# crowsonkb/style-transfer-pytorch

Hardware: AMD Instinct MI355X
Metric: optimizer iterations/sec (higher is better)
Workload: dtype f32 (3x3 convs: fp16x3 split-plane MFMA, fp32 accumulate); 1 GPU; 512x512 single-scale hot loop (closure + Adam + clamp + EMA), 1 style image 512x512, VGG-19 synthetic weights, max pooling; parallelism=single GPU

## Files before the change

include/st_amd.h:

```cpp
#ifndef ST_AMD_H
#define ST_AMD_H

#ifdef __cplusplus
extern "C" {
#endif

#define ST_AMD_ABI_VERSION 2

#define ST_NUM_CONVS 13
#define ST_NUM_STYLE_LAYERS 5
#define ST_CONTENT_LAYER 22
#define ST_NUM_LOSS_TERMS 7

enum st_pooling { ST_POOL_MAX = 0, ST_POOL_AVERAGE = 1, ST_POOL_L2 = 2 };

typedef struct st_net st_net;
typedef struct st_plan st_plan;

const char* st_last_error(void);
int st_abi_version(void);
const char* st_compiled_arch(void);
int st_has_experiments(void);
int st_env_switches(const char** names, int capacity);
int st_set_option(const char* name, int value, int clear);
// ... 70 lines not shown

typedef struct st_exchange {
    int kind;
    long long count;
    float* send_up;
    float* send_down;
    float* recv_up;
    float* recv_down;
    float* buffer;
    int root;
    int channel;
    void* stream;
} st_exchange;
int st_plan_create_strip(st_plan** out, const st_net* net, int global_height, int width, int row_begin,
                         int row_end);
int st_plan_set_rank(st_plan* plan, int rank, int world);
int st_plan_closure_begin(st_plan* plan, const float* image, float* grad_out);
int st_plan_closure_next(st_plan* plan, st_exchange* exchange, void* stream);

typedef struct st_fabric st_fabric;
int st_fabric_unique_id(unsigned char* id128);
int st_fabric_create(st_fabric** out, const unsigned char* id_trunk128, const unsigned char* id_heads128, int rank, int world,
                     int self_halo);
int st_fabric_destroy(st_fabric* fabric);
int st_fabric_abort(st_fabric* fabric);
int st_fabric_selftest(st_fabric* fabric, void* stream, int timeout_ms);
int st_plan_closure_run(st_plan* plan, st_fabric* fabric, void* stream);
long long st_qn_strip_state_bytes(long long count, int world);
int st_qn_strip_dots(void* state, long long count, int rank, int world, const float* grad, st_exchange* gather,
                     void* stream);
int st_qn_strip_apply(void* state, long long count, int world, float* image, const float* grad, float* ema_value,
                      double ema_decay, void* stream);
int st_plan_qn_strip_step(st_plan* plan, st_fabric* fabric, float* image, float* grad, void* state, float* ema_value,
                          double ema_decay, void* stream);
int st_plan_losses(st_plan* plan, float** losses);
int st_plan_term_losses(st_plan* plan, float** terms, int* count);
int st_plan_forward_begin(st_plan* plan, const float* image, int last_layer);
int st_plan_moment_sums(st_plan* plan, int layer, float* sums, void* stream);

int st_plan_set_graph(st_plan* plan, int enable);

int st_plan_profile_enable(st_plan* plan, int enable);
int st_plan_profile_read(st_plan* plan, long long* launches, double* millis, double* flops);
int st_plan_profile_read_hbm(st_plan* plan, int category, long long* launches, double* millis, double* bytes);

int st_op_sqrtm_ns(const float* a, float* root, int n, void* stream);
int st_op_sqrtm_ns_backward(const float* root, const float* grad_root, float* grad_a, int n, void* stream);
int st_op_sqrtm_ns_backward_diag(const float* root, float grad_diag, float* grad_a, int n, void* stream);
int st_op_tv_loss(const float* image, int height, int width, float* loss_out, float* grad_out, void* stream);
int st_op_conv3x3(const float* in, const float* weight, const float* bias, float* out, int cin, int cout,
                  int height, int width, int relu, int precision, void* stream);
int st_op_conv3x3_dgrad(const float* grad_out, const float* relu_out, const float* weight, float* grad_in,
                        int cin, int cout, int height, int width, int precision, void* stream);
int st_op_conv3x3_strip(const float* in, const float* halo, int has_up, int has_down, const float* weight,
                        const float* bias, float* out, int cin, int cout, int height, int width, int relu, int dgrad,
                        int precision, void* stream);
int st_op_conv3x3_strip_ex(const float* in, const float* halo, int has_up, int has_down, const float* weight,
                           const float* bias, float* out, const float* out_mask, int cin, int cout, int height, int width,
                           int relu, int dgrad, int accumulate, int overlap, int precision, void* stream);

int st_op_conv1x1(const float* in, const float* weight, const float* bias, float* out, int cin, int cout,
                  long long npix, int precision, void* stream);

int st_op_pool2x2(const float* in, float* out, int channels, int height, int width, int mode, void* stream);
int st_op_pool2x2_backward(const float* in, const float* grad_out, float* grad_in, int channels, int height, int width,
                           int mode, void* stream);


typedef struct st_head st_head;
int st_head_create(st_head** out, int kind, int channels, int height, int width, int precision);
int st_head_destroy(st_head* head);
long long st_head_device_bytes(const st_head* head);
long long st_head_state_floats(const st_head* head);
int st_head_moments(st_head* head, const float* feat, float* mean_out, float* srm_out, void* stream);
int st_head_forward(st_head* head, const float* feat, const float* mean_t, const float* cov_t, const float* root_t,
                    const float* gram_t, float eps, float* loss_out, float* state, void* stream);
int st_head_backward(st_head* head, const float* feat, const float* state, const float* upstream, float* grad_feat,
                     void* stream);

long long st_op_reduce_scratch_floats(void);
int st_op_mse_loss(const float* x, const float* target, long long count, float* scratch, float* loss_out, void* stream);
int st_op_mse_loss_backward(const float* x, const float* target, long long count, const float* upstream, float* grad,
                            void* stream);
int st_op_scaled_mse_loss(const float* x, const float* target, long long count, float eps, float* scratch, float* totals,
                          float* loss_out, void* stream);
int st_op_scaled_mse_loss_backward(const float* x, const float* target, long long count, const float* totals,
                                   const float* upstream, float* grad, void* stream);
int st_op_tv_value(const float* image, int height, int width, float* scratch, float* loss_out, void* stream);
int st_op_tv_loss_backward(const float* image, int height, int width, const float* upstream, float* grad, void* stream);


int st_op_sqrtm_time(int n, int iters, double* fwd_us, double* bwd_us, void* stream);

int st_op_conv3x3_time(int cin, int cout, int height, int width, int dgrad, int precision, int iters,
                       double* avg_us, void* stream);

int st_op_mfma_rate(int lds_reads, int waves, int steps, int launches, double* tflops, double* mhz, void* stream);

int st_op_mfma_valu_rate(int lds_reads, int waves, int steps, int launches, int valu_waves, int valu_steps,
                         int valu_prio, double* tflops, double* mhz, double* cycles, void* stream);

int st_op_winograd_consumer_rate(int steps, int launches, double* tflops, void* stream);

int st_plan_debug_read(st_plan* plan, int what, float* out, int count);

int st_op_grid_barrier_time(int workgroups, int rounds, int payload_floats, int groups, double* us_per_round, int* errors,
                            void* stream);

#ifdef __cplusplus
}
#endif
#endif
```

style-transfer-pytorch_amd/csrc/st_api.hip:

```cpp
#include <atomic>
#include <cmath>
#include <cstdlib>
#include <cstring>
#include <mutex>
#include <vector>

#include "st_plan.h"

namespace st {

static thread_local std::string g_error;
void set_error(const char* fmt, ...) {
    char buf[1024];
    va_list ap;
    va_start(ap, fmt);
    vsnprintf(buf, sizeof(buf), fmt, ap);
    va_end(ap);
    g_error = buf;
}
const char* get_error() { return g_error.c_str(); }

static std::mutex g_option_mutex;
static std::vector<std::pair<std::string, int>> g_option_override;
static std::atomic<unsigned> g_option_gen{1};
// ... 467 lines not shown
        if (p->net->conv_elem == 1) { tail.zero = reinterpret_cast<unsigned int*>(p->amax_word); tail.zero_count = 64ll * kAmaxWordUints; }
    }
    const AdamScalars sc = adam_scalars(step, lr, beta1, beta2, eps, ema_decay);
    FoldUpdate upd{image, exp_avg, exp_avg_sq, ema_value, sc, tail};
    if (upd.tail.losses_copy == upd.tail.losses8) upd.tail.losses_copy = nullptr;
    p->defer_sum = fold_tail;
    p->fold_update = fold_step ? &upd : nullptr;
    p->fold_updated = false;
    const int closure_rc = closure_entry(p, image, p->grad_img, losses_out, s);
    p->defer_sum = false;
    p->fold_update = nullptr;
    if (closure_rc) return 1;
    if (p->fold_updated) {
        p->fold_updated = false;
        p->amax_clean = tail.zero != nullptr;
        return 0;
    }
    const int rc = hbm_profiled(p, HBM_ADAM, 9.0 * 3 * 4.0 * p->H * p->W, s, [&] {
        return launch_adam_clamp_ema(image, p->grad_img, exp_avg, exp_avg_sq, ema_value, 3ll * p->H * p->W, sc, s, tail);
    });
    p->amax_clean = rc == 0 && tail.zero != nullptr;
    return rc;
}

int st_plan_apply_update(st_plan* p, float* image, const float* grad, float* exp_avg, float* exp_avg_sq,
                         float* ema_value, long long step, double lr, double beta1, double beta2, double eps,
                         double ema_decay, void* stream) {
    ST_REQUIRE(p && image && grad && exp_avg && exp_avg_sq && ema_value, "st_plan_apply_update: null argument");
    ST_REQUIRE(step >= 1, "st_plan_apply_update: step must be >= 1");
    return launch_adam_clamp_ema(image, grad, exp_avg, exp_avg_sq, ema_value, 3ll * p->H * p->W,
                                 adam_scalars(step, lr, beta1, beta2, eps, ema_decay),
                                 static_cast<hipStream_t>(stream));
}

int st_plan_debug_read(st_plan* p, int what, float* out, int count) {
    ST_REQUIRE(p && out && count > 0, "st_plan_debug_read: bad argument");
    const bool grad_map = what >= 16 && what < 16 + kNumOps;
    ST_REQUIRE((what == 0 && count <= 4 * kStreamBlocks) || (what == 1 && count <= kStreamBlocks * 256 * 5 && tv_debug_buffer()) ||
                   (what == 2 && count == 64) ||
                   (grad_map && p->grads_allocated && (size_t)count == node_at(p, what - 16).count()),
               "st_plan_debug_read: unknown buffer or count out of range");
    ST_HIP(hipDeviceSynchronize());
    if (what == 2) {
        std::vector<unsigned int> words((size_t)64 * kAmaxWordUints);
        ST_HIP(hipMemcpy(words.data(), p->amax_word, words.size() * sizeof(unsigned int), hipMemcpyDeviceToHost));
        for (int w = 0; w < 64; ++w) {
            unsigned int m = 0;
            for (int slot = 0; slot < kAmaxSlots; ++slot) m = std::max(m, words[(size_t)w * kAmaxWordUints + (size_t)slot * kAmaxSlotStride]);
            memcpy(&out[w], &m, sizeof(float));
        }
        return 0;
    }
    if (grad_map) {
        ST_HIP(hipMemcpy(out, node_at(p, what - 16).g, (size_t)count * sizeof(float), hipMemcpyDeviceToHost));
        return 0;
    }
    ST_HIP(hipMemcpy(out, what == 0 ? p->red_partials : tv_debug_buffer(), (size_t)count * sizeof(float), hipMemcpyDeviceToHost));
    return 0;
}

int st_plan_losses(st_plan* p, float** losses) {
    ST_REQUIRE(p && losses, "st_plan_losses: null argument");
    *losses = p->losses;
    return 0;
}

int st_plan_moment_sums(st_plan* p, int layer, float* sums, void* stream) {
    ST_REQUIRE(p && sums, "st_plan_moment_sums: null argument");
    int idx = -1;
    for (int k = 0; k < p->n_style; ++k)
        if (kProgram[p->style_op[k]].feat_index == layer) idx = k;
    ST_REQUIRE(idx >= 0, "st_plan_moment_sums: features[%d] is not a style layer", layer);
    if (ensure_style_alloc(p, p->head[p->style_op[idx]], p->style_kind[idx])) return 1;
    return moment_sums_of_tap(p, idx, sums, static_cast<hipStream_t>(stream));
}

int st_plan_set_graph(st_plan* p, int enable) {
    ST_REQUIRE(p, "st_plan_set_graph: null plan");
    p->graph_enabled = enable != 0;
    if (!enable) invalidate_graph(p);
    return 0;
}

int st_plan_profile_enable(st_plan* p, int enable) {
    ST_REQUIRE(p, "st_plan_profile_enable: null plan");
    p->profiling = enable != 0;
    return 0;
}

int st_plan_profile_read(st_plan* p, long long* launches, double* millis, double* flops) {
    ST_REQUIRE(p, "st_plan_profile_read: null plan");
    for (size_t i = 0; i < p->events_used; ++i) {
        ProfileEvent& e = p->events[i];
        ST_HIP(hipEventSynchronize(e.stop));
        float ms = 0.f;
        ST_HIP(hipEventElapsedTime(&ms, e.start, e.stop));
        p->prof_ms += ms;
        p->prof_flops += e.flops;
        p->prof_launches += 1;
    }
    p->events_used = 0;
    p->hbm_used = 0;
    if (launches) *launches = p->prof_launches;
    if (millis) *millis = p->prof_ms;
    if (flops) *flops = p->prof_flops;
    p->prof_launches = 0;
    p->prof_ms = 0;
    p->prof_flops = 0;
    return 0;
}
// ... 24 lines not shown
```

style-transfer-pytorch_amd/csrc/st_closure.hip:

```cpp
#include <cmath>
#include <cstdlib>
#include <mutex>

#include "st_plan.h"

namespace st {

void conv_arithmetic(const st_net* net, int conv, bool dgrad, ConvProblem& c) {
    const bool wide = dgrad ? net->wide_bwd[conv] : net->wide_fwd[conv];
    if (wide) {
        c.wgt_split = dgrad ? net->wsx_bwd[conv] : net->wsx_fwd[conv];
        c.planes = 3;
        c.elem = 0;
    } else {
        c.wgt_split = dgrad ? net->ws_bwd[conv] : net->ws_fwd[conv];
        c.planes = net->conv_planes;
        c.elem = net->conv_elem;
    }
}

int plan_alloc(st_plan* p, float** out, size_t floats) {
    void* ptr = nullptr;
    const size_t bytes = ((floats * sizeof(float) + 255) / 256) * 256;
    hipError_t e = hipMalloc(&ptr, bytes);
// ... 448 lines not shown
    return 0;
}

static bool head5_masks_its_gradient() {
    static Option opt("ST_HEAD5_MASK", 1);
    return opt.get() != 0;
}

int style_head_gradient(st_plan* p, const HeadSite& at, hipStream_t s) {
    StyleHead& h = *at.h;
    const Node& tap = *at.tap;
    const bool f16 = p->net->conv_elem == 1;
    static Option head_f32("ST_HEAD_1X1_F32", 0);
    const float* out_mask = (at.slot == 4 && head5_masks_its_gradient()) ? tap.y : nullptr;
    if (ablate_side() & 2) return 0;
    return hbm_profiled(p, HBM_HEAD_1X1, 2.0 * h.n * (double)tap.h * tap.w * sizeof(float), s, [&] {
        return head_step(h, tap.y, tap.h, tap.w, at.grad, s, f16 && !head_f32.get(), tap.y_amax, f16 ? at.grad_amax : nullptr, out_mask);
    });
}

bool op_is_tap(const st_plan* p, int op) {
    for (int i = 0; i < p->n_content; ++i)
        if (p->content_op[i] == op) return true;
    for (int k = 0; k < p->n_style; ++k)
        if (p->style_op[k] == op) return true;
    return false;
}

int join_head_for_conv(st_plan* p, int conv_index, hipStream_t s) {
    for (int k = 0; k < p->n_style; ++k) {
        if (!head_taps_conv(p, k, conv_index)) continue;
        ST_HIP(hipStreamWaitEvent(s, p->head_done[k], 0));
    }
    return 0;
}

void dgrad_conv(const st_plan* p, int i, ConvProblem& c) {
    const st_net* net = p->net;
    const OpDesc& op = kProgram[i];
    const OpDesc& pop = kProgram[i - 1];
    const Node& n = p->conv[op.index];
    const Node& in = node_at(p, i - 1);
    const bool top = i == kNumOps - 1;
    c.in = n.g; c.mask = (top && !head5_masks_its_gradient()) ? n.y : nullptr;
    c.out_mask = (pop.kind == 0) ? in.y : nullptr;
    c.wgt = net->w_bwd[op.index]; c.bias = nullptr; c.out = in.g;
    c.cin = op.cout; c.cout = op.cin; c.height = n.h; c.width = n.w; c.taps = 9; c.relu = 0;
    c.accumulate = (pop.kind == 0 && op_is_tap(p, i - 1)) ? 1 : 0;
    c.scratch = p->conv_scratch;
    conv_arithmetic(net, op.index, true, c);
    c.amax_word = n.g_amax; c.out_amax = net->conv_elem == 1 ? in.g_amax : nullptr;
}

int run_backward(st_plan* p, float* grad_image, hipStream_t s) {
    const st_net* net = p->net;
    for (int i = kNumOps - 1; i >= 0; --i) {
        const OpDesc& op = kProgram[i];
        if (op.kind == 0) {
            Node& n = p->conv[op.index];
            if (join_head_for_conv(p, op.index, s)) return 1;
            if (op.index == 0) {
                ST_HIP(hipStreamWaitEvent(s, p->tv_done, 0));
                if (hbm_profiled(p, HBM_CONV1_DGRAD, (64 + 3 + 3) * 4.0 * p->H * p->W, s, [&] {
                        return launch_conv_first_dgrad(n.g, nullptr, net->w_first, grad_image, p->dp_scratch, p->H, p->W, 1, s, nullptr, 0, 0,
                                                       p->dp_parts, p->fold_update);
                    }))
                    return 1;
                p->fold_updated = p->fold_update != nullptr;
                continue;
            }
            const OpDesc& pop = kProgram[i - 1];
            if (pop.kind == 0 && join_head_for_conv(p, pop.index, s)) return 1;
            if (i - 1 == p->content_op[0]) ST_HIP(hipStreamWaitEvent(s, p->content_done, 0));
            ConvProblem c{};
            dgrad_conv(p, i, c);
            if (conv_launch_profiled(p, c, s)) return 1;
        } else {
            Node& n = p->pool[op.index];
            const OpDesc& pop = kProgram[i - 1];
            Node& in = p->conv[pop.index];
            const double bytes = in.coded ? (in.count() + 1.25 * n.count()) * 4.0 : (2.0 * in.count() + n.count()) * 4.0;
            if (hbm_profiled(p, HBM_POOL_BWD, bytes, s, [&] {
                    if (in.coded) return launch_pool_bwd_codes(in.pool_code, n.g, in.g, in.c, in.h, in.w, s);
                    return launch_pool_bwd(in.y, n.g, in.g, in.c, in.h, in.w, net->pooling, s);
                }))
                return 1;
        }
    }
    return 0;
}

int run_tap_backward(st_plan* p, const float* const* seed, float* grad_image, hipStream_t s, bool onto_image) {
    const st_net* net = p->net;
    const bool bounds = net->conv_elem == 1;
    int top = -1;
    for (int i = 0; i < kNumOps; ++i)
        if (seed[i]) top = i;
    ST_REQUIRE(top >= 0, "st_plan_backward: no tap gradient given");
    if (bounds)
        ST_HIP(hipMemsetAsync(reinterpret_cast<unsigned int*>(p->amax_word) + (size_t)16 * kAmaxWordUints, 0,
                              (size_t)32 * kAmaxWordUints * sizeof(unsigned int), s));
    {
        Node& n = node_at(p, top);
        if (launch_seed_grad(seed[top], kProgram[top].kind == 0 ? n.y : nullptr, n.g, (long long)n.count(), 0,
                             bounds ? n.g_amax : nullptr, s))
            return 1;
    }
    for (int i = top; i >= 0; --i) {
        const OpDesc& op = kProgram[i];
        if (op.kind == 0 && op.index == 0) {
            if (hbm_profiled(p, HBM_CONV1_DGRAD, (64 + 3 + (onto_image ? 3 : 0)) * 4.0 * p->H * p->W, s, [&] {
                    return launch_conv_first_dgrad(p->conv[0].g, nullptr, net->w_first, grad_image, p->dp_scratch, p->H, p->W,
                                                   onto_image ? 1 : 0, s, nullptr, 0, 0, p->dp_parts,
                                                   onto_image ? p->fold_update : nullptr);
                }))
                return 1;
            if (onto_image) p->fold_updated = p->fold_update != nullptr;
            return 0;
        }
        Node& in = node_at(p, i - 1);
        const float* in_seed = seed[i - 1];
        if (op.kind == 0) {
            if (in_seed && launch_seed_grad(in_seed, nullptr, in.g, (long long)in.count(), 0, nullptr, s)) return 1;
            ConvProblem c{};
            dgrad_conv(p, i, c);
            c.mask = nullptr;
            c.accumulate = in_seed ? 1 : 0;
            if (conv_launch_profiled(p, c, s)) return 1;
        } else {
            Node& n = p->pool[op.index];
            if (hbm_profiled(p, HBM_POOL_BWD, (2.0 * in.count() + n.count()) * 4.0, s, [&] {
                    return launch_pool_bwd(in.y, n.g, in.g, in.c, in.h, in.w, net->pooling, s);
                }))
                return 1;
            if (in_seed && launch_seed_grad(in_seed, in.y, in.g, (long long)in.count(), 1, bounds ? in.g_amax : nullptr, s))
                return 1;
        }
    }
    return 0;
}

static bool shallow_heads_lockstep(const st_plan* p) {
    static Option opt("ST_HEAD_LOCKSTEP", 1);
    return opt.get() != 0 && p->net->conv_elem == 1;
}

int require_targets(const st_plan* p) {
    for (int i = 0; i < p->n_content; ++i)
        ST_REQUIRE(p->content_set[p->content_op[i]], "content target %d (features[%d]) not set (st_plan_set_content_target_at)", i,
                   kProgram[p->content_op[i]].feat_index);
    for (int j = 0; j < p->n_style; ++j)
        ST_REQUIRE(p->head[p->style_op[j]].target_set, "style target %d (features[%d]) not set (st_plan_set_style_target)", j,
                   kProgram[p->style_op[j]].feat_index);
    for (int r = 1; r < p->n_regions; ++r)
        for (int j = 0; j < p->n_style; ++j)
            ST_REQUIRE(p->region_head[r - 1][p->style_op[j]].target_set,
                       "style target %d (features[%d]) of region %d not set (st_plan_set_region_style_target)", j,
                       kProgram[p->style_op[j]].feat_index, r);
    return 0;
}

int loss_and_grad(st_plan* p, const float* image, float* grad_out, float* losses_out, hipStream_t s) {
    if (require_targets(p) || ensure_grad_alloc(p)) return 1;
    if (ensure_streams(p, s)) return 1;
    if (p->timeline) ST_HIP(hipEventRecord(p->tl_start, s));
    auto tv = [&](hipStream_t ts) {
        return hbm_profiled(p, HBM_TV, 2.0 * 3 * 4.0 * p->H * p->W, ts, [&] {
            return launch_tv(image, p->H, p->W, p->tv_weight, grad_out, p->red_partials, p->losses + 6, ts, p->tickets + 0);
        });
    };
    static Option tv_slot_opt("ST_TV_SLOT", 0);
    const bool tv_tail = tv_slot_opt.get() == 1 && !p->aux_stream;
    if (!tv_tail) {
        const int tvk = shallow_heads_lockstep(p) ? 2 : 0;
        if (!p->aux_stream && ensure_head_stream(p, tvk)) return 1;
        hipStream_t tvs = p->aux_stream ? p->aux_stream : p->head_stream[tvk];
        ST_HIP(hipEventRecord(p->aux_in, s));
        ST_HIP(hipStreamWaitEvent(tvs, p->aux_in, 0));
        if (tv(tvs)) return 1;
        ST_HIP(hipEventRecord(p->tv_done, tvs));
    }
    if (run_forward(p, image, 29, s, true)) return 1;
    if (p->timeline) ST_HIP(hipEventRecord(p->tl_fwd, s));
// ... 106 lines not shown
```

style-transfer-pytorch_amd/csrc/st_common.h:

```cpp
#pragma once

#include <hip/hip_runtime.h>

#include <algorithm>
#include <atomic>
#include <cstdarg>
#include <cstdio>
#include <string>

namespace st {

typedef float f32x16 __attribute__((ext_vector_type(16)));
typedef float f32x4 __attribute__((ext_vector_type(4)));
typedef float f32x2 __attribute__((ext_vector_type(2)));

constexpr int kWave = 64;

void set_error(const char* fmt, ...);
const char* get_error();

#define ST_HIP(expr)                                                                           \
    do {                                                                                       \
        hipError_t _e = (expr);                                                                \
        if (_e != hipSuccess) {                                                                \
// ... 71 lines not shown
};
__device__ __forceinline__ float w2_gdiag(const W2LossJob& j) { return -2.f * (j.weight / (float)j.n); }
__device__ __forceinline__ void w2_loss_block(const W2LossJob& j, float* scratch) {
#pragma clang fp contract(off)
    float sm = 0.f, sc = 0.f;
    for (int i = threadIdx.x; i < j.n; i += 256) {
        const float d = j.mean[i] - j.mean_t[i];
        sm += d * d;
        const size_t ii = (size_t)i * j.n + i;
        sc += (j.cov_t[ii] + j.cov[ii]) - 2.f * j.root[ii];
    }
    sm = block_sum_256(sm, scratch);
    sc = block_sum_256(sc, scratch);
    if (threadIdx.x == 0) {
        const float fn = (float)j.n;
        j.loss_out[0] = (sm / fn + sc / fn) * j.weight;
        j.gdiag_out[0] = w2_gdiag(j);
    }
}

static inline int ceil_div(int a, int b) { return (a + b - 1) / b; }

struct ConvProblem {
    const float* in;
    const float* mask;
    const float* wgt;
    const float* bias;
    float* out;
    int cin, cout, height, width;
    int taps;
    int relu;
    int accumulate;
    float* scratch;
    const float* in_halo;
    int has_up, has_down;
    int tune;
    const void* wgt_split;
    int planes;
    int elem;
    unsigned int* amax_word;
    int amax_measure;
    int halo_amax_folded;
    const unsigned int* halo_bound_up;
    const unsigned int* halo_bound_down;
    const unsigned int* wgt_amax;
    const float* out_mask;
    unsigned int* out_amax;
    int row_begin, row_end;
    int row_skip_begin, row_skip_len;
    int xcd_co_groups;
    int overlap_part;
    float* pool_out;
    unsigned char* pool_code;
    const void* wgt_wino;
    int wino;
};
constexpr int kAmaxSlots = 32;
constexpr int kAmaxSlotStride = 64;
constexpr int kAmaxWordUints = kAmaxSlots * kAmaxSlotStride;
#if defined(__HIPCC__)
__device__ __forceinline__ void amax_commit(unsigned int m, unsigned int* bound) {
#pragma unroll
    for (int off = 32; off >= 1; off >>= 1) {
        const unsigned int o = (unsigned int)__shfl_xor((int)m, off);
        m = o > m ? o : m;
    }
    unsigned int* slot = bound + (blockIdx.x % kAmaxSlots) * kAmaxSlotStride;
    if ((threadIdx.x & 63) == 0 && (m >> 23) > (*slot >> 23)) atomicMax(slot, m);
}
__device__ __forceinline__ unsigned int amax_read(const unsigned int* bound) {
    unsigned int m = bound[(threadIdx.x % kAmaxSlots) * kAmaxSlotStride];
#pragma unroll
    for (int off = 16; off >= 1; off >>= 1) {
        const unsigned int o = (unsigned int)__shfl_xor((int)m, off);
        m = o > m ? o : m;
    }
    return (unsigned int)__builtin_amdgcn_readfirstlane((int)m);
}
__device__ __forceinline__ unsigned int logical_block(int remap) {
    const unsigned int linear = blockIdx.y * gridDim.x + blockIdx.x, total = gridDim.x * gridDim.y;
    if (!remap || (total & 7u) != 0) return linear;
    return (linear & 7u) * (total >> 3) + (linear >> 3);
}
__device__ __forceinline__ unsigned int abs_bits(float v) { return __builtin_bit_cast(unsigned int, v) & 0x7fffffffu; }
__device__ __forceinline__ unsigned int amax_with_halo(unsigned int own, const unsigned int* up, const unsigned int* down) {
    if (up) { const unsigned int u = up[0] & 0x7fffffffu; own = u > own ? u : own; }
    if (down) { const unsigned int d = down[0] & 0x7fffffffu; own = d > own ? d : own; }
    return own;
}
__host__ __device__ __forceinline__ int scale_exp(unsigned int amax_bits) {
    const int ef = (int)((amax_bits >> 23) & 0xffu);
    if (ef == 0 || ef == 255) return 0;
    const int e = 14 - (ef - 126);
    return e > 120 ? 120 : (e < -120 ? -120 : e);
}
__device__ __forceinline__ float pow2f(int e) { return __builtin_bit_cast(float, (unsigned int)(127 + e) << 23); }
#endif
int launch_conv_split(const ConvProblem& p, hipStream_t stream);
#if defined(ST_EXPERIMENTS)
size_t winograd_weight_bytes(int cin, int cout);
int launch_winograd_weights(const float* w_torch, void* out, int cin, int cout, int dgrad, hipStream_t s);
bool conv_wino_applies(const ConvProblem& p);
bool conv_wino_preferred(const ConvProblem& p);
int launch_conv_wino(const ConvProblem& p, hipStream_t s);
#else
inline size_t winograd_weight_bytes(int, int) { return 256; }
inline int launch_winograd_weights(const float*, void*, int, int, int, hipStream_t) {
    set_error("the Winograd convolution (precision code 5) needs a library built with build.py --experiments");
    return 1;
}
inline bool conv_wino_applies(const ConvProblem&) { return false; }
inline bool conv_wino_preferred(const ConvProblem&) { return false; }
inline int launch_conv_wino(const ConvProblem&, hipStream_t) { return launch_winograd_weights(nullptr, nullptr, 0, 0, 0, nullptr); }
#endif
int launch_amax(const float* x, long long n, unsigned int* word, int single, hipStream_t s);
bool conv_pc_applies(const ConvProblem& p);
bool conv_pc_preferred(const ConvProblem& p);
int launch_conv_pc(const ConvProblem& p, hipStream_t stream);
bool conv_fat_applies(const ConvProblem& p);
bool conv_fat_preferred(const ConvProblem& p);
int launch_conv_fat(const ConvProblem& p, hipStream_t stream);
bool conv1x1_split_applies(const ConvProblem& p);
int launch_conv1x1_split(const ConvProblem& p, hipStream_t stream);
int launch_conv_splitk_reduce(const ConvProblem& p, int ksplit, hipStream_t stream);
inline bool conv_precision_valid(int code) { return code == 0 || code == 2 || code == 3 || code == 4; }
inline int conv_precision_planes(int code) { return code == 4 ? 2 : code; }
inline int conv_precision_elem(int code) { return code == 4 ? 1 : 0; }
inline size_t split_weight_bytes(int cin, int cout, int planes) { return (size_t)cin * cout * 9 * 2 * planes + 256; }
int launch_relayout_split(const float* w, void* out, int cin, int cout, int dgrad, int planes, int elem, hipStream_t s);
constexpr size_t kConvScratchFloats = (size_t)8 << 20;
int launch_conv(const ConvProblem& p, hipStream_t stream);
double conv_flops(const ConvProblem& p);

int launch_relayout_fwd(const float* w, float* out, int cin, int cout, hipStream_t stream);
int launch_relayout_dgrad(const float* w, float* out, int cin, int cout, hipStream_t stream);

constexpr int kPackScratchUints = 2 * 512 * 8 + 64;
int launch_pack_rows(const float* src, const float* mask, int channels, int height, int width, float* out_up,
                     float* out_down, hipStream_t s, unsigned int* bounds_up = nullptr, unsigned int* bounds_down = nullptr,
                     unsigned int* scratch = nullptr);

int launch_conv_first_fwd(const float* image, const float* w , const float* b, float* out,
                          int height, int width, hipStream_t stream, const float* halo = nullptr,
                          int has_up = 0, int has_down = 0, unsigned int* out_amax = nullptr);
bool conv_first_gram_applies(int height, int width, const float* image, const float* out, int max_splits);
int launch_conv_first_fwd_gram(const float* image, const float* w, const float* b, float* out, int height, int width,
                               hipStream_t stream, unsigned int* out_amax, float* partial, float* partial_sum, int max_splits,
                               int* splits, float w_l1max, float b_max);
int conv_first_dgrad_parts(int height, int width);
struct FoldUpdate;
int launch_conv_first_dgrad(const float* grad_out, const float* relu_out, const float* w, float* grad_image,
                            float* dp_scratch, int height, int width, int accumulate, hipStream_t stream,
                            const float* ghalo = nullptr, int has_up = 0, int has_down = 0, int parts = 1,
                            const FoldUpdate* update = nullptr);

int launch_pool_fwd(const float* in, float* out, int channels, int height, int width, int mode, hipStream_t s);
bool conv_pc_fuses_pool(const ConvProblem& p);
int fold_halo_amax(const ConvProblem& p, hipStream_t stream);
struct PcOverlap {
    int rows_b;
    int rows_bottom;
    int shape_i, tw_i;
    int shape_b, tw_b;
    double cost_split, cost_whole;
    bool pays;
    bool pool;
};
bool conv_pc_overlap_choice(const ConvProblem& p, PcOverlap* out);
int launch_pool_bwd_codes(const unsigned char* code, const float* grad_out, float* grad_in, int channels, int height,
                          int width, hipStream_t s);
// ... 273 lines not shown
```

style-transfer-pytorch_amd/csrc/st_conv.hip:

```cpp
#include <cstdlib>
#include <type_traits>

#include "st_common.h"

namespace st {

namespace {

constexpr int kChunk3x3 = 8, kChunk1x1 = 32;

template <int TAPS, int TW, int WN, int WGM>
struct Cfg {
    static constexpr int KC = (TAPS == 9) ? kChunk3x3 : kChunk1x1;
    static constexpr int WGN = 4 / WGM;
    static constexpr int TCO = 64 * WGM;
    static constexpr int NPIX = 32 * WN * WGN;
    static constexpr int TH = NPIX / TW;
    static constexpr int HALO = (TAPS == 9) ? 1 : 0;
    static constexpr int LH = TH + 2 * HALO;
    static constexpr int LW = TW + 2 * HALO;
    static constexpr int PLANE = LH * LW;
    static constexpr int NE_IN = KC * PLANE;
    static constexpr int IN_FLOATS = (NE_IN + 3) & ~3;
    static constexpr int NI = (NE_IN + 255) / 256;
// ... 358 lines not shown

long long padded_area(int h, int w, int th, int tw) {
    return (long long)ceil_div(h, th) * th * (long long)ceil_div(w, tw) * tw;
}

template <int WN, int WGM>
int launch_3x3(const ConvProblem& p, int ksplit, hipStream_t s) {
    constexpr int NPIX = 32 * WN * (4 / WGM);
    int best = 32;
    long long best_area = padded_area(p.height, p.width, NPIX / 32, 32);
    for (int tw : {16, 8}) {
        const long long a = padded_area(p.height, p.width, NPIX / tw, tw);
        if (a < best_area) { best_area = a; best = tw; }
    }
    if (best == 32) return launch_cfg<9, 32, WN, WGM>(p, ksplit, s);
    if (best == 16) return launch_cfg<9, 16, WN, WGM>(p, ksplit, s);
    return launch_cfg<9, 8, WN, WGM>(p, ksplit, s);
}

}

int launch_conv_splitk_reduce(const ConvProblem& p, int ksplit, hipStream_t stream) {
    const long long total = (long long)p.cout * p.height * p.width;
    const int hw = p.height * p.width;
    const bool aligned = ((reinterpret_cast<uintptr_t>(p.out) | reinterpret_cast<uintptr_t>(p.out_mask)) & 15) == 0;
    if (hw % 4 == 0 && aligned) {
        const int rblocks = (int)std::min<long long>((total / 4 + 255) / 256, 4096);
        hipLaunchKernelGGL(conv_splitk_reduce_kernel<4>, dim3(rblocks), dim3(256), 0, stream, p.scratch, p.bias, p.out,
                           p.cout, hw, ksplit, p.relu, p.accumulate, p.out_amax, p.out_mask);
    } else {
        const int rblocks = (int)std::min<long long>((total + 255) / 256, 4096);
        hipLaunchKernelGGL(conv_splitk_reduce_kernel<1>, dim3(rblocks), dim3(256), 0, stream, p.scratch, p.bias, p.out,
                           p.cout, hw, ksplit, p.relu, p.accumulate, p.out_amax, p.out_mask);
    }
    ST_LAUNCH_CHECK();
    return 0;
}

double conv_flops(const ConvProblem& p) {
    return 2.0 * p.taps * (double)p.cin * p.cout * (double)p.height * p.width;
}

static int env_int(const char* name, int dflt) {
    const char* v = option_env(name);
    return v ? atoi(v) : dflt;
}

int launch_conv(const ConvProblem& p_in, hipStream_t stream) {
    ConvProblem p = p_in;
    if (p.tune == 0) p.tune = env_int("ST_CONV_TUNE", 0);
    ST_REQUIRE(p.taps == 9 || p.taps == 1, "conv: taps must be 9 or 1");
    if (p.planes > 0 && p.taps == 9 && p.wgt_split && p.cin % 16 == 0)
        return launch_conv_split(p, stream);
    const int KC = (p.taps == 9) ? kChunk3x3 : kChunk1x1;
    ST_REQUIRE(p.cin % KC == 0 && p.cout % 64 == 0, "conv: Cin %% %d and Cout %% 64 required (got %d, %d)", KC,
               p.cin, p.cout);
    ST_REQUIRE((long long)p.height * p.width * KC * 4 < (1ll << 31), "conv: image too large for 32-bit tile maps");
    const long long pixels = (long long)p.height * p.width;
    const int co_tiles = p.cout / 64;
    const long long wg_a = ((pixels + 255) / 256) * co_tiles;
    const long long wg_b = ((pixels + 127) / 128) * co_tiles;
    int shape = (wg_a >= 512) ? 0 : 1;
    if (pixels <= 64 && p.cout % 128 == 0) shape = 2;
    long long wgs = shape == 0 ? wg_a : (shape == 1 ? wg_b : ((pixels + 63) / 64) * (p.cout / 128));
    const int force_shape = env_int("ST_CONV_SHAPE", -1);
    if (force_shape >= 0 && (force_shape != 2 || p.cout % 128 == 0)) {
        shape = force_shape;
        wgs = shape == 0 ? wg_a : (shape == 1 ? wg_b : ((pixels + 63) / 64) * (p.cout / 128));
    }
    int ksplit = 1;
    const int force_ks = env_int("ST_CONV_KSPLIT", -1);
    if (force_ks >= 1 && p.scratch && (p.cin / KC) % force_ks == 0 &&
        (size_t)force_ks * p.cout * pixels <= kConvScratchFloats) {
        ksplit = force_ks;
    } else if (p.scratch && shape != 0) {
        const int nchunks = p.cin / KC;
        const int min_chunks = (p.taps == 9) ? 4 : 1;
        while (wgs * ksplit * 2 <= 640 && nchunks % (ksplit * 2) == 0 && nchunks / (ksplit * 2) >= min_chunks &&
               (size_t)(ksplit * 2) * p.cout * pixels <= kConvScratchFloats)
            ksplit *= 2;
    }
    if (ksplit == 1 && env_int("ST_CONV1X1_FP32", 0) == 0 && conv1x1_split_applies(p)) return launch_conv1x1_split(p, stream);
    if (p.taps == 1) {
        ConvProblem q = p;
        q.height = 1;
        q.width = (int)pixels;
        if (shape == 0) return launch_cfg<1, 256, 2, 1>(q, ksplit, stream);
        if (shape == 1) return launch_cfg<1, 128, 1, 1>(q, ksplit, stream);
        return launch_cfg<1, 64, 1, 2>(q, ksplit, stream);
    }
    if (shape == 0) return launch_3x3<2, 1>(p, ksplit, stream);
    if (shape == 1) return launch_3x3<1, 1>(p, ksplit, stream);
    return launch_3x3<1, 2>(p, ksplit, stream);
}

namespace {
template <int VEC, bool BOUND>
__global__ __launch_bounds__(256) void pack_rows_kernel(const float* __restrict__ src,
                                                        const float* __restrict__ mask, int H, int W,
                                                        float* __restrict__ out_up,
                                                        float* __restrict__ out_down, unsigned int* __restrict__ bound_up,
                                                        unsigned int* __restrict__ bound_down, unsigned int* __restrict__ scratch,
                                                        int ticket_at, int rows_total, int rows_per_block) {
    const int wave = threadIdx.x >> 6, lane = threadIdx.x & 63;
    unsigned int m_up = 0, m_down = 0;
    const int r_end = min(rows_total, ((int)blockIdx.x + 1) * rows_per_block);
// ... 141 lines not shown
```

style-transfer-pytorch_amd/csrc/st_conv_fat.hip:

```cpp
#include "st_common.h"

namespace st {
namespace {

typedef _Float16 f16x8 __attribute__((ext_vector_type(8)));
typedef unsigned int u32x4 __attribute__((ext_vector_type(4)));
typedef unsigned int u32x2 __attribute__((ext_vector_type(2)));
constexpr int SK = 16;
constexpr int kOOR = 0x40000000;

template <int B, int E, typename F>
__device__ __forceinline__ void sfor(F&& f) {
    if constexpr (B < E) {
        f(std::integral_constant<int, B>{});
        sfor<B + 1, E>(f);
    }
}

__device__ __forceinline__ float bload(__amdgpu_buffer_rsrc_t rs, int voff, int soff) {
    return __builtin_bit_cast(float, __builtin_amdgcn_raw_buffer_load_b32(rs, voff, soff, 0));
}
constexpr int waitcnt_imm(int vm, int lgkm) { return (vm & 15) | ((vm >> 4) << 14) | (7 << 4) | ((lgkm & 15) << 8); }

template <int CB>
// ... 251 lines not shown
            coded ? p.pool_code + (size_t)co_base * (PH * PW) : reinterpret_cast<unsigned char*>(out_base), 0, coded ? 32 * PH * PW : 0, 0x00020000);
        __builtin_amdgcn_wave_barrier();
#pragma unroll
        for (int j = 0; j < 4; ++j)
#pragma unroll
            for (int r = 0; r < 16; ++r) slab[((r & 3) + 8 * (r >> 2) + 4 * half) * TP + j * 32 + l31] = acc[i][j][r] * unscale;
        __builtin_amdgcn_wave_barrier();
        const unsigned off0 = inb ? (unsigned)((lrow * H + y) * W + x) * 4u : 0x7FFFFFFFu;
        const unsigned step = (unsigned)(2 * HW) * 4u;
        const unsigned poff0 = pin ? (unsigned)((lrow * PH + (y >> 1)) * PW + (x >> 1)) * 4u : 0x7FFFFFFFu;
        const unsigned pstep = (unsigned)(2 * PH * PW) * 4u;
        const float* slab_rd = slab + lrow * TP + k * 4;
        f32x4 o_next = {0.f, 0.f, 0.f, 0.f}, m_next = {0.f, 0.f, 0.f, 0.f};
        if constexpr (RMW) {
            o_next = __builtin_bit_cast(f32x4, __builtin_amdgcn_raw_buffer_load_b128(os_ld, (int)off0, 0, 0));
            m_next = __builtin_bit_cast(f32x4, __builtin_amdgcn_raw_buffer_load_b128(ms_ld, (int)off0, 0, 0));
        }
#pragma unroll 4
        for (int q = 0; q < 16; ++q) {
            const int off = (int)(off0 + (unsigned)q * step);
            f32x4 v = *reinterpret_cast<const f32x4*>(slab_rd + q * (2 * TP));
            const float bvv = __builtin_bit_cast(float, __builtin_amdgcn_raw_buffer_load_b32(bs, (2 * q + lrow) * 4, 0, 0));
            const f32x4 o = o_next, m = m_next;
            if constexpr (RMW) {
                const int off1 = (q + 1 < 16) ? (int)(off0 + (unsigned)(q + 1) * step) : 0x7FFFFFFF;
                o_next = __builtin_bit_cast(f32x4, __builtin_amdgcn_raw_buffer_load_b128(os_ld, off1, 0, 0));
                m_next = __builtin_bit_cast(f32x4, __builtin_amdgcn_raw_buffer_load_b128(ms_ld, off1, 0, 0));
                __builtin_amdgcn_sched_barrier(0);
            }
#pragma unroll
            for (int e = 0; e < 4; ++e) {
                float x_ = fmaxf(v[e] + bvv, relu_floor);
                if constexpr (RMW) {
                    x_ += o[e];
                    x_ = (m[e] > mask_thr) ? x_ : 0.f;
                }
                v[e] = x_;
            }
            if (RMW || !coded) __builtin_amdgcn_raw_buffer_store_b128(__builtin_bit_cast(u32x4, v), os, off, 0, 0);
            if constexpr (!RMW) {
                if (pool) {
                    float m0 = fmaxf(v[0], v[1]), m1 = fmaxf(v[2], v[3]);
                    const int mine = (v[1] > v[0] ? 1 : 0) | (v[3] > v[2] ? 2 : 0);
                    const float n0 = __builtin_bit_cast(float, __builtin_amdgcn_update_dpp(0, __builtin_bit_cast(int, m0), 0x128, 0xf, 0xf, false));
                    const float n1 = __builtin_bit_cast(float, __builtin_amdgcn_update_dpp(0, __builtin_bit_cast(int, m1), 0x128, 0xf, 0xf, false));
                    const int theirs = __builtin_amdgcn_update_dpp(0, mine, 0x128, 0xf, 0xf, false);
                    const int at0 = n0 > m0 ? 2 + (theirs & 1) : (mine & 1);
                    const int at1 = n1 > m1 ? 2 + ((theirs >> 1) & 1) : ((mine >> 1) & 1);
                    m0 = fmaxf(m0, n0);
                    m1 = fmaxf(m1, n1);
                    const unsigned poff = poff0 + (unsigned)q * pstep;
                    const f32x2 pv = {m0, m1};
                    __builtin_amdgcn_raw_buffer_store_b64(__builtin_bit_cast(u32x2, pv), ps, (int)poff, 0, 0);
                    const int two = (at0 | (m0 > 0.f ? 4 : 0)) | ((at1 | (m1 > 0.f ? 4 : 0)) << 8);
                    __builtin_amdgcn_raw_buffer_store_b16((unsigned short)two, cs, pin ? (int)(poff >> 2) : 0x7FFFFFFF, 0, 0);
                }
            }
            amax_e = max(amax_e, inb ? max(max(abs_bits(v[0]), abs_bits(v[1])), max(abs_bits(v[2]), abs_bits(v[3]))) : 0u);
        }
    });
    if (p.out_amax && !partial) amax_commit(amax_e, p.out_amax);
}

template <int CB, bool RMW, int TUNE = 0>
int launch_fat_cfg(const ConvProblem& p, int ksplit, hipStream_t s) {
    using C = FCfg<CB>;
    auto kern = conv_fat_kernel<CB, RMW, TUNE>;
    static bool attr = false;
    if (!attr) {
        ST_HIP(hipFuncSetAttribute(reinterpret_cast<const void*>(kern), hipFuncAttributeMaxDynamicSharedMemorySize, C::LDS));
        attr = true;
    }
    const int tiles_x = ceil_div(p.width, C::TW), tiles_y = ceil_div(p.height, C::TH);
    const int n_co = p.cout / C::TCO;
    const long long total = (long long)tiles_x * tiles_y * n_co * ksplit;
    ST_REQUIRE(total > 0 && total < (1ll << 30), "conv (fat tile): grid out of range");
    hipLaunchKernelGGL(kern, dim3((unsigned)total), dim3(256), C::LDS, s, p, tiles_x, n_co, ksplit, p.cin / SK / ksplit, (int)total);
    ST_LAUNCH_CHECK();
    if (ksplit > 1) return launch_conv_splitk_reduce(p, ksplit, s);
    return 0;
}

}

bool conv_fat_applies(const ConvProblem& p) {
    return p.taps == 9 && p.planes == 2 && p.elem == 1 && p.wgt_split && p.amax_word && !p.mask && !p.in_halo && p.cin % SK == 0 &&
           p.cout % 64 == 0 && p.width % 4 == 0 && p.row_begin == 0 && p.row_end == 0 && p.row_skip_len == 0 && p.overlap_part == 0 &&
           ((reinterpret_cast<uintptr_t>(p.out) | reinterpret_cast<uintptr_t>(p.out_mask) | reinterpret_cast<uintptr_t>(p.pool_out)) & 15) == 0 &&
           (long long)SK * p.height * p.width * 4 < (long long)kOOR && (long long)p.height * p.width * 32 * 4 < (1ll << 31) &&
           (long long)9 * (p.cin / SK) * p.cout * 32 * 2 < (1ll << 31);
}

static int fat_n_cu() {
    static std::atomic<int> cached[16];
    int dev = 0;
    if (hipGetDevice(&dev) != hipSuccess || dev < 0 || dev >= 16) return 256;
    int cus = cached[dev].load(std::memory_order_relaxed);
    if (cus) return cus;
    if (hipDeviceGetAttribute(&cus, hipDeviceAttributeMultiprocessorCount, dev) != hipSuccess || cus < 8) cus = 256;
    cached[dev].store(cus, std::memory_order_relaxed);
    return cus;
}

bool conv_fat_preferred(const ConvProblem& p) {
    static Option fat_opt("ST_CONV_FAT", 1);
    const int mode = fat_opt.get();
    if (mode == 0 || !conv_fat_applies(p)) return false;
    if (mode == 2) return true;
// ... 29 lines not shown
```

style-transfer-pytorch_amd/csrc/st_conv_pc.hip:

```cpp
#include <mutex>
#include <type_traits>

#include "st_common.h"

#ifndef ST_PC_WDMA_ALL
#define ST_PC_WDMA_ALL 1
#endif

namespace st {
namespace {

typedef _Float16 f16x8 __attribute__((ext_vector_type(8)));
constexpr int SK = 16;
constexpr int kOOR = 0x40000000;

template <int B, int E, typename F>
__device__ __forceinline__ void sfor(F&& f) {
    if constexpr (B < E) {
        f(std::integral_constant<int, B>{});
        sfor<B + 1, E>(f);
    }
}

__device__ __forceinline__ float bload(__amdgpu_buffer_rsrc_t rs, int voff, int soff) {
    return __builtin_bit_cast(float, __builtin_amdgcn_raw_buffer_load_b32(rs, voff, soff, 0));
}

__device__ __forceinline__ void amax_commit_lean(unsigned int m, unsigned int* bound) {
    sfor<0, 5>([&](auto K) __attribute__((always_inline)) {
        constexpr int k = 1 << decltype(K)::value;
        const unsigned int o = (unsigned int)__builtin_amdgcn_ds_swizzle((int)m, (k << 10) | 0x1f);
        m = o > m ? o : m;
    });
    const unsigned int o = (unsigned int)__builtin_amdgcn_ds_bpermute((int)(((threadIdx.x & 63) ^ 32) << 2), (int)m);
    m = o > m ? o : m;
    unsigned int* slot = bound + (blockIdx.x % kAmaxSlots) * kAmaxSlotStride;
    if ((threadIdx.x & 63) == 0 && (m >> 23) > (*slot >> 23)) atomicMax(slot, m);
}

template <int TW, int WN, int CW>
struct PCfg {
    static constexpr bool XL = CW == 8;
    static constexpr bool WDMA = ST_PC_WDMA_ALL ? true : XL;
    static constexpr int PT = (WN == 1 && !XL) ? 512 : 256;
    static constexpr int THREADS = 64 * CW + PT;
    static constexpr int SETS = XL ? 1 : 2;
    static constexpr int TCO = 64;
    static constexpr int NPIX = 32 * WN * CW;
    static constexpr int TH = NPIX / TW;
    static constexpr int LH = TH + 2, LW = TW + 2;
    static constexpr int NPX = LH * LW;
    static constexpr int ACT_PLANE = NPX * 32;
    static constexpr int W_PLANE = 9 * TCO * 32;
    static constexpr int BUF = 2 * (ACT_PLANE + W_PLANE);
    static constexpr int W_OFF = 2 * ACT_PLANE;
    static constexpr int NIT = (2 * NPX + PT - 1) / PT;
    static constexpr int NWP = 9 * TCO * 2;
    static constexpr int NWT = (NWP + PT - 1) / PT;
};

template <int TW, int WN, int CW, bool HALO>
__global__ __launch_bounds__((CW == 8 || WN == 1 ? 768 : 512), 1) void conv_pc_kernel(ConvProblem p, int tiles_x, int n_co_tiles, int ksplit,
                                                         int nchunks, int total) {
    using C = PCfg<TW, WN, CW>;
    extern __shared__ __attribute__((aligned(16))) unsigned char smem[];
    const int tid = threadIdx.x, lane = tid & 63;
    const int wave = __builtin_amdgcn_readfirstlane(tid >> 6);
    const bool producer = wave >= CW;
    const int cwave = wave;
    const int wn = cwave;
    const int ptid = tid - 64 * CW;
    const int l31 = lane & 31, half = lane >> 5;
    const int H = p.height, W = p.width, HW = H * W;
    const int Y0 = p.row_begin, Y1 = p.row_end ? p.row_end : H;

    const int my_tiles = (total - (int)blockIdx.x + (int)gridDim.x - 1) / (int)gridDim.x;
    const int gtot = my_tiles * nchunks;
    struct Tile { int x0, y0, co0, kslice; };
    auto tile_of = [&](int ordinal) __attribute__((always_inline)) {
        const int v = blockIdx.x + ordinal * gridDim.x;
        int bid = ((total & 7) == 0) ? (v & 7) * (total >> 3) + (v >> 3) : v;
        Tile t;
        if (p.xcd_co_groups > 1) {
            const int G = p.xcd_co_groups, x = v & 7, L = v >> 3;
            const int nw = n_co_tiles * ksplit, wpg = nw / G, w_local = L % wpg, pl = L / wpg;
            const int ppg = (total >> 3) / wpg;
            const int wt = (x % G) * wpg + w_local;
            t.co0 = (wt % n_co_tiles) * C::TCO;
            t.kslice = wt / n_co_tiles;
            bid = (x / G) * ppg + pl;
        } else {
            t.co0 = (bid % n_co_tiles) * C::TCO;
            bid /= n_co_tiles;
            t.kslice = bid % ksplit;
            bid /= ksplit;
        }
        t.x0 = (bid % tiles_x) * TW;
        t.y0 = Y0 + (bid / tiles_x) * C::TH;
        if (p.row_skip_len != 0 && t.y0 >= p.row_skip_begin) t.y0 += p.row_skip_len;
        return t;
    };

    const unsigned char* wsplit = static_cast<const unsigned char*>(p.wgt_split);
    const size_t w_plane_stride = (size_t)9 * (p.cin / SK) * p.cout * 32;
    const size_t w_tap_stride = (size_t)(p.cin / SK) * p.cout * 32;
    const int ea = scale_exp(amax_with_halo(amax_read(p.amax_word), p.halo_bound_up, p.halo_bound_down));
    const int ew = scale_exp(*reinterpret_cast<const unsigned int*>(wsplit + 2 * w_plane_stride));
    const float in_scale = pow2f(ea), out_scale_a = pow2f(-ea), out_scale_w = pow2f(-ew);

    const bool stamp = (p.tune & 32) != 0 && ksplit == 1 && p.scratch != nullptr;
    unsigned long long t_a = 0, t_b = 0, t_c = 0, t_prev = 0, t_begin = 0, r_begin = 0;
    if (stamp) {
        t_begin = t_prev = __builtin_amdgcn_s_memtime();
        r_begin = __builtin_amdgcn_s_memrealtime();
    }
    auto mark = [&](unsigned long long& bucket) __attribute__((always_inline)) {
        if (stamp) {
            const unsigned long long t = __builtin_amdgcn_s_memtime();
            bucket += t - t_prev;
            t_prev = t;
        }
    };

    if (producer) {
        if (C::XL && !(p.tune & 128)) __builtin_amdgcn_s_setprio(3);
        int goff[C::NIT], aoff[C::NIT];
        int hoff[HALO ? C::NIT : 1];
        bool halo_tile = false;
        bool set_halo[C::SETS][2] = {};
        int l_tile = 0, l_chunk = 0, l_chunk0 = 0, l_co0 = 0;
        auto point_at_tile = [&](int ordinal) __attribute__((always_inline)) {
            const Tile t = tile_of(ordinal);
            l_chunk0 = t.kslice * nchunks;
            l_co0 = t.co0;
            bool any_halo = false;
#pragma unroll
            for (int i = 0; i < C::NIT; ++i) {
                const int it = (ptid + i * C::PT < 2 * C::NPX) ? ptid + i * C::PT : 2 * C::NPX - 1;
                const int g = it / C::NPX, q = it % C::NPX;
                const int y = t.y0 - 1 + q / C::LW, x = t.x0 - 1 + q % C::LW;
                const bool ok = y >= 0 && y < H && x >= 0 && x < W;
                goff[i] = ok ? (8 * g * HW + y * W + x) * 4 : kOOR;
                aoff[i] = q * 32 + ((g ^ ((q >> 3) & 1)) * 16);
                if constexpr (HALO) {
                    const bool xin = x >= 0 && x < W;
                    const bool top = xin && y == -1 && p.has_up, bot = xin && y == H && p.has_down;
                    hoff[i] = top ? (8 * g * W + x) * 4 : (bot ? ((p.cin + 8 * g) * W + x) * 4 : kOOR);
                    any_halo = any_halo || top || bot;
                }
            }
            if constexpr (HALO) halo_tile = __builtin_amdgcn_ballot_w64(any_halo) != 0;
        };
        float ract[C::SETS][C::NIT][8];
        float rhal[HALO ? C::SETS : 1][HALO ? C::NIT : 1][8];
        f32x4 rwt[C::SETS][2][C::NWT];
        const int chunk_bytes = SK * HW * 4;
        int loaded = 0;
        constexpr int NA = C::NIT / 2;
        const bool ablate_prod = (p.tune & 256) != 0;
        const bool ablate_loads = (p.tune & 1024) != 0, ablate_stores = (p.tune & 2048) != 0;
        auto load_part = [&](auto SET, auto PART, auto WITHW) __attribute__((always_inline)) {
            constexpr int st = decltype(SET)::value, part = decltype(PART)::value;
            constexpr bool withw = decltype(WITHW)::value;
            if (ablate_prod || ablate_loads) return;
            const int cc = l_chunk0 + l_chunk;
            const __amdgpu_buffer_rsrc_t rs = __builtin_amdgcn_make_buffer_rsrc(
                const_cast<float*>(p.in) + (size_t)cc * SK * HW, 0, chunk_bytes, 0x00020000);
            sfor<(part == 1 ? NA : 0), (part == 0 ? NA : C::NIT)>([&](auto I) __attribute__((always_inline)) {
                constexpr int i = decltype(I)::value;
#pragma unroll
                for (int c = 0; c < 8; ++c) ract[st][i][c] = bload(rs, goff[i], c * HW * 4);
            });
            if constexpr (HALO) {
                if constexpr (part != 1) set_halo[st][0] = halo_tile;
                if constexpr (part != 0) set_halo[st][1] = halo_tile;
                if (halo_tile) {
                    const __amdgpu_buffer_rsrc_t hs = __builtin_amdgcn_make_buffer_rsrc(
                        const_cast<float*>(p.in_halo) + (size_t)cc * SK * W, 0, (p.cin + SK) * W * 4, 0x00020000);
                    sfor<(part == 1 ? NA : 0), (part == 0 ? NA : C::NIT)>([&](auto I) __attribute__((always_inline)) {
                        constexpr int i = decltype(I)::value;
#pragma unroll
                        for (int c = 0; c < 8; ++c) rhal[st][i][c] = bload(hs, hoff[i], c * W * 4);
                    });
                }
            }
            sfor<(part == 1 ? 1 : 0), (!withw ? 0 : part == 0 ? 1 : 2)>([&](auto PL) __attribute__((always_inline)) {
                constexpr int pl = decltype(PL)::value;
                sfor<0, C::NWT>([&](auto I) __attribute__((always_inline)) {
                    constexpr int i = decltype(I)::value;
                    const int f = (ptid + i * C::PT < C::NWP) ? ptid + i * C::PT : C::NWP - 1;
                    const int tap = f / (C::TCO * 2), r = f % (C::TCO * 2);
                    rwt[st][pl][i] = *reinterpret_cast<const f32x4*>(wsplit + pl * w_plane_stride + tap * w_tap_stride +
                                                                     ((size_t)cc * p.cout + l_co0) * 32 + r * 16);
                });
            });
        };
        auto advance = [&]() __attribute__((always_inline)) {
            if (++l_chunk == nchunks) {
                l_chunk = 0;
                if (++l_tile < my_tiles) point_at_tile(l_tile);
            }
        };
        constexpr std::integral_constant<int, 0> PA{};
        constexpr std::integral_constant<int, 1> PB{};
        constexpr std::integral_constant<int, 2> PALL{};
        constexpr std::integral_constant<bool, !C::WDMA> WL{};
        constexpr std::integral_constant<bool, !C::WDMA> WW{};
        auto load_next = [&](auto SET, auto WITHW) __attribute__((always_inline)) {
            if (loaded >= gtot) return;
            ++loaded;
            load_part(SET, PALL, WITHW);
            advance();
        };
        auto store_part = [&](auto SET, auto PART, unsigned char* buf, auto WITHW) __attribute__((always_inline)) {
            constexpr int st = decltype(SET)::value, part = decltype(PART)::value;
            constexpr bool withw = decltype(WITHW)::value;
            if (ablate_prod || ablate_stores) return;
            sfor<(part == 1 ? NA : 0), (part == 0 ? NA : C::NIT)>([&](auto I) __attribute__((always_inline)) {
                constexpr int i = decltype(I)::value;
                f16x8 h0, h1;
#pragma unroll
                for (int c = 0; c < 8; ++c) {
                    float v = ract[st][i][c];
                    if constexpr (HALO) {
                        if (set_halo[st][i < NA ? 0 : 1]) v += rhal[st][i][c];
                    }
                    v *= in_scale;
                    const _Float16 a = (_Float16)v;
                    h0[c] = a;
                    h1[c] = (_Float16)(v - (float)a);
                }
                *reinterpret_cast<f16x8*>(buf + aoff[i]) = h0;
                *reinterpret_cast<f16x8*>(buf + C::ACT_PLANE + aoff[i]) = h1;
            });
            sfor<(part == 1 ? 1 : 0), (!withw ? 0 : part == 0 ? 1 : 2)>([&](auto PL) __attribute__((always_inline)) {
                constexpr int pl = decltype(PL)::value;
                sfor<0, C::NWT>([&](auto I) __attribute__((always_inline)) {
                    constexpr int i = decltype(I)::value;
                    const int f = (ptid + i * C::PT < C::NWP) ? ptid + i * C::PT : C::NWP - 1;
                    const int row = f >> 1, hsel = f & 1;
                    *reinterpret_cast<f32x4*>(buf + C::W_OFF + pl * C::W_PLANE + row * 32 +
                                              ((hsel ^ ((row >> 3) & 1)) * 16)) = rwt[st][pl][i];
                });
            });
        };
        auto store_chunk = [&](auto SET, unsigned char* buf, auto WITHW) __attribute__((always_inline)) {
            store_part(SET, PALL, buf, WITHW);
        };
        constexpr std::integral_constant<int, 0> S0{};
        constexpr std::integral_constant<int, C::SETS - 1> S1{};
        point_at_tile(0);
        load_next(S0, WW);
        store_chunk(S0, smem, WW);
        load_next(S0, WL);
        if constexpr (C::SETS == 2) load_next(S1, WL);
        mark(t_a);
        __syncthreads();
        mark(t_b);
        if constexpr (C::SETS == 2) {
            for (int g = 0; g < gtot; g += 2) {
                if (g + 1 < gtot) {
                    store_chunk(S0, smem + C::BUF, WL);
                    load_next(S0, WL);
                }
                mark(t_a);
                __syncthreads();
                mark(t_b);
                if (g + 1 >= gtot) break;
                if (g + 2 < gtot) {
                    store_chunk(S1, smem, WL);
                    load_next(S1, WL);
                }
                mark(t_a);
                __syncthreads();
                mark(t_b);
            }
        } else {
            int left = nchunks;
            for (int g = 0; g < gtot; ++g) {
                if (g + 1 < gtot) {
                    unsigned char* img = smem + ((g + 1) & 1) * C::BUF;
                    const bool more = g + 2 < gtot;
                    store_part(S0, PA, img, WL);
                    if (more) load_part(S0, PA, WL);
                    store_part(S0, PB, img, WL);
                    if (more) {
// ... 207 lines not shown
                const unsigned poff0 = pin ? (unsigned)((int)lrow * (PH * PW) + (y >> 1) * PW + (x >> 1)) * 4u : 0x7FFFFFFFu;
                const unsigned pstep = (unsigned)(RG * PH * PW) * 4u;
                f32x4 o_next = {0.f, 0.f, 0.f, 0.f}, m_next = {0.f, 0.f, 0.f, 0.f};
                if constexpr (loads) {
                    o_next = __builtin_bit_cast(f32x4, __builtin_amdgcn_raw_buffer_load_b128(os_ld, (int)off0, 0, 0));
                    m_next = __builtin_bit_cast(f32x4, __builtin_amdgcn_raw_buffer_load_b128(ms_ld, (int)off0, 0, 0));
                    const f32x4 nothing = {0.f, 0.f, 0.f, 0.f};
                    __builtin_amdgcn_raw_buffer_store_b128(
                        __builtin_bit_cast(__attribute__((__vector_size__(4 * sizeof(unsigned int)))) unsigned int, nothing), os, 0x7FFFFFFF, 0, 0);
                }
#pragma unroll(C::XL ? 2 : 4 * WN)
                for (int q4 = 0; q4 < 4 * WN; ++q4) {
                    const int off = (int)(off0 + (unsigned)q4 * step);
                    f32x4 v = *reinterpret_cast<const f32x4*>(slab_rd + q4 * (RG * TP));
                    const float bv = bias_rd[q4 * RG];
                    const f32x4 o = o_next, m = m_next;
                    if constexpr (loads) {
                        const int off1 = (q4 + 1 < 4 * WN) ? (int)(off0 + (unsigned)(q4 + 1) * step) : 0x7FFFFFFF;
                        o_next = __builtin_bit_cast(f32x4, __builtin_amdgcn_raw_buffer_load_b128(os_ld, off1, 0, 0));
                        m_next = __builtin_bit_cast(f32x4, __builtin_amdgcn_raw_buffer_load_b128(ms_ld, off1, 0, 0));
                        __builtin_amdgcn_sched_barrier(0);
                    }
#pragma unroll
                    for (int e = 0; e < 4; ++e) {
                        float x_ = v[e] + bv;
                        if (relu) x_ = fmaxf(x_, 0.f);
                        if constexpr (loads) {
                            if (accumulate) x_ += o[e];
                            if (out_mask) x_ = (m[e] > 0.f) ? x_ : 0.f;
                        }
                        v[e] = x_;
                        amax = max(amax, inb ? abs_bits(x_) : 0u);
                    }
                    if (loads || !coded)
                        __builtin_amdgcn_raw_buffer_store_b128(
                            __builtin_bit_cast(__attribute__((__vector_size__(4 * sizeof(unsigned int)))) unsigned int, v), os, off, 0, 0);
                    if constexpr (WN == 2 && TW == 32 && !loads) {
                        if (pool) {
                            float m0 = fmaxf(v[0], v[1]), m1 = fmaxf(v[2], v[3]);
                            const int mine = (v[1] > v[0] ? 1 : 0) | (v[3] > v[2] ? 2 : 0);
                            const float n0 = __builtin_bit_cast(float, __builtin_amdgcn_update_dpp(0, __builtin_bit_cast(int, m0), 0x128, 0xf, 0xf, false));
                            const float n1 = __builtin_bit_cast(float, __builtin_amdgcn_update_dpp(0, __builtin_bit_cast(int, m1), 0x128, 0xf, 0xf, false));
                            const int theirs = __builtin_amdgcn_update_dpp(0, mine, 0x128, 0xf, 0xf, false);
                            const int at0 = n0 > m0 ? 2 + (theirs & 1) : (mine & 1);
                            const int at1 = n1 > m1 ? 2 + ((theirs >> 1) & 1) : ((mine >> 1) & 1);
                            m0 = fmaxf(m0, n0);
                            m1 = fmaxf(m1, n1);
                            const unsigned poff = poff0 + (unsigned)q4 * pstep;
                            typedef float f32x2 __attribute__((ext_vector_type(2)));
                            f32x2 pv = {m0, m1};
                            __builtin_amdgcn_raw_buffer_store_b64(
                                __builtin_bit_cast(__attribute__((__vector_size__(2 * sizeof(unsigned int)))) unsigned int, pv), ps, (int)poff, 0, 0);
                            if (coded) {
                                const int two = (at0 | (m0 > 0.f ? 4 : 0)) | ((at1 | (m1 > 0.f ? 4 : 0)) << 8);
                                __builtin_amdgcn_raw_buffer_store_b16((unsigned short)two, cs, pin ? (int)(poff >> 2) : 0x7FFFFFFF, 0, 0);
                            }
                        }
                    }
                }
            } else {
                __builtin_amdgcn_wave_barrier();
#pragma unroll
                for (int j = 0; j < WN; ++j) {
                    const int pix = (wn * WN + j) * 32 + l31_e;
                    const int y = t.y0 + pix / TW, x = t.x0 + pix % TW;
                    const bool inb = (y < Y1) && (x < W);
                    const int pix_bytes = inb ? (y * W + x) * 4 : 0x7FFFFFFF;
                    auto offset_r = [&](int r) __attribute__((always_inline)) {
                        const int row = (r & 3) + 8 * (r >> 2) + 4 * half_e;
                        return inb ? row * HW * 4 + pix_bytes : 0x7FFFFFFF;
                    };
                    float o_next = 0.f, m_next = 0.f;
                    if constexpr (loads) {
                        o_next = __builtin_bit_cast(float, __builtin_amdgcn_raw_buffer_load_b32(os_ld, offset_r(0), 0, 0));
                        m_next = __builtin_bit_cast(float, __builtin_amdgcn_raw_buffer_load_b32(ms_ld, offset_r(0), 0, 0));
                    }
#pragma unroll
                    for (int r = 0; r < 16; ++r) {
                        const int row = (r & 3) + 8 * (r >> 2) + 4 * half_e;
                        const int off = offset_r(r);
                        const float o = o_next, mk = m_next;
                        if constexpr (loads) {
                            const int off1 = (r + 1 < 16) ? offset_r(r + 1) : 0x7FFFFFFF;
                            o_next = __builtin_bit_cast(float, __builtin_amdgcn_raw_buffer_load_b32(os_ld, off1, 0, 0));
                            m_next = __builtin_bit_cast(float, __builtin_amdgcn_raw_buffer_load_b32(ms_ld, off1, 0, 0));
                            __builtin_amdgcn_sched_barrier(0);
                        }
                        float v = acc[i][j][r] * out_scale_a * out_scale_w;
                        v += bias_w[i * 32 + row];
                        if (relu) v = fmaxf(v, 0.f);
                        if constexpr (loads) {
                            if (accumulate) v += o;
                            if (out_mask) v = (mk > 0.f) ? v : 0.f;
                        }
                        __builtin_amdgcn_raw_buffer_store_b32(__builtin_bit_cast(unsigned int, v), os, off, 0, 0);
                        amax = max(amax, inb ? abs_bits(v) : 0u);
                    }
                }
            }
            };
            if (accumulate || out_mask) store_rows(std::true_type{});
            else store_rows(std::false_type{});
        }
        if (C::XL && k + 1 < my_tiles) __syncthreads();
        mark(t_c);
    }
    if (p.out_amax && !partial) amax_commit_lean(amax, p.out_amax);
    if (stamp && cwave == 0 && lane == 0) {
        __builtin_amdgcn_s_waitcnt(0);
        mark(t_c);
        unsigned long long* dst = reinterpret_cast<unsigned long long*>(p.scratch) + (size_t)blockIdx.x * 8;
        dst[0] = t_a;
        dst[1] = t_b;
        dst[2] = t_c;
        dst[5] = __builtin_amdgcn_s_memtime() - t_begin;
        dst[7] = __builtin_amdgcn_s_memrealtime() - r_begin;
        dst[6] = 1;
    }
}

inline int ceil_div_i(int a, int b) { return (a + b - 1) / b; }

template <int TW, int WN, int CW, bool HALO>
int launch_pc_cfg_h(const ConvProblem& p, int ksplit, hipStream_t stream) {
    using C = PCfg<TW, WN, CW>;
    constexpr int LDS = 2 * C::BUF + (C::XL ? CW * 64 : CW * (32 * (WN * 32 + 8) + 64)) * 4;
    static_assert(!C::XL || CW * 32 * (WN * 32 + 8) * 4 <= C::BUF, "XL epilogue slabs must fit one image");
    static_assert(LDS <= 160 * 1024, "LDS budget of one CU");
    static bool attr_set = false;
    static int n_cu = 256;
    auto kern = conv_pc_kernel<TW, WN, CW, HALO>;
    if (!attr_set) {
        ST_HIP(hipFuncSetAttribute(reinterpret_cast<const void*>(kern), hipFuncAttributeMaxDynamicSharedMemorySize, LDS));
        int dev = 0;
        hipDeviceProp_t prop;
        if (hipGetDevice(&dev) == hipSuccess && hipGetDeviceProperties(&prop, dev) == hipSuccess && prop.multiProcessorCount >= 8)
            n_cu = prop.multiProcessorCount & ~7;
        attr_set = true;
    }
    const int rows = (p.row_end ? p.row_end : p.height) - p.row_begin - p.row_skip_len;
    ST_REQUIRE(p.row_skip_len == 0 || (p.row_skip_begin - p.row_begin) % C::TH == 0,
               "conv (producer/consumer): the skipped row range must start on a tile row");
    const int tiles_x = ceil_div_i(p.width, TW), tiles_y = ceil_div_i(rows, C::TH);
    const int n_co_tiles = p.cout / C::TCO;
    const long long total = (long long)tiles_x * tiles_y * n_co_tiles * ksplit;
    ST_REQUIRE(total > 0 && total < (1ll << 30), "conv grid out of range");
    static Option spare_opt("ST_STRIP_SPARE_CUS", 0);
    int cus = n_cu;
    if (p.overlap_part == 1 && spare_opt.get() > 0 && n_cu - spare_opt.get() >= 64) cus = (n_cu - spare_opt.get()) & ~7;
    const int grid = total <= cus ? (int)total : cus;
    ConvProblem q = p;
    q.xcd_co_groups = 1;
    {
        static Option cg_opt("ST_CONV_XCD_COGROUPS", 0);
        const long long px_tiles = (long long)tiles_x * tiles_y;
        if ((total & 7) == 0 && grid == n_cu && cus == n_cu && n_cu % 8 == 0 && cg_opt.get() != 1) {
            const double wbytes = 9.0 * p.cin * p.cout * 4.0, abytes = (double)p.cin * rows * p.width * 4.0;
            double best = wbytes * 8.0 + abytes;
            for (int G = 2; G <= 8; G *= 2) {
                if ((n_co_tiles * ksplit) % G != 0 || px_tiles % (8 / G) != 0) continue;
                const double cost = wbytes * 8.0 / G + abytes * G;
                if (cg_opt.get() == G || (cg_opt.get() == 0 && cost < 0.9 * best)) {
                    best = cost;
                    q.xcd_co_groups = G;
                }
            }
        }
    }
    hipLaunchKernelGGL(kern, dim3((unsigned)grid), dim3(C::THREADS), LDS, stream, q, tiles_x, n_co_tiles, ksplit,
                       p.cin / SK / ksplit, (int)total);
    ST_LAUNCH_CHECK();
    if (ksplit > 1) {
        ST_REQUIRE(p.row_begin == 0 && p.row_end == 0, "conv (producer/consumer): K split needs the whole image");
        return launch_conv_splitk_reduce(p, ksplit, stream);
    }
    return 0;
}

template <int TW, int WN, int CW>
int launch_pc_cfg(const ConvProblem& p, int ksplit, hipStream_t stream) {
    if (p.in_halo) return launch_pc_cfg_h<TW, WN, CW, true>(p, ksplit, stream);
    return launch_pc_cfg_h<TW, WN, CW, false>(p, ksplit, stream);
}

template <int WN, int CW>
int launch_pc_tw(const ConvProblem& p, int ksplit, hipStream_t s, int tw) {
    if (tw == 32) return launch_pc_cfg<32, WN, CW>(p, ksplit, s);
    if (tw == 16) return launch_pc_cfg<16, WN, CW>(p, ksplit, s);
    return launch_pc_cfg<8, WN, CW>(p, ksplit, s);
}

}

bool conv_pc_applies(const ConvProblem& p) {
    static Option halo_ok("ST_CONV_PC_HALO", 1);
    return p.taps == 9 && p.planes == 2 && p.elem == 1 && p.wgt_split && p.amax_word && !p.mask &&
           (!p.in_halo || halo_ok.get()) && p.cin % SK == 0 && p.cout % 64 == 0;
}

namespace {
bool xl_tile_pays(const ConvProblem& p) {
    static Option xl_opt("ST_CONV_PC_XL", 1);
    const int xl = xl_opt.get();
    const long long tiles = (long long)ceil_div_i(p.width, 32) * ceil_div_i(p.height, 16) * (p.cout / 64);
    return xl && p.cin >= 64 && tiles >= 256;
}
}

bool conv_pc_preferred(const ConvProblem& p) {
    if (!conv_pc_applies(p)) return false;
    static Option model_opt("ST_CONV_PC_MODEL", 1);
    if (model_opt.get()) return true;
    const long long pixels = (long long)p.height * p.width;
    const long long wg_a = ((pixels + 255) / 256) * (p.cout / 64);
    return xl_tile_pays(p) || (p.cin >= 256 && wg_a < 512);
}

namespace {
struct PcChoice { int shape, tw, ksplit; double cost; int split_row, shape2, tw2; };

constexpr double kPcLaunch = 2.31;
constexpr double kPcChunk[4] = {0.0, 3.972, 2.607, 1.706};
constexpr double kPcRound[4] = {0.0, 13.369, 8.402, 4.379};
constexpr double kPcReduce0 = 2.995, kPcReduce1 = 1.163e-6;
constexpr int kPcPix[4] = {0, 512, 256, 128};

PcChoice choose_pc_single(const ConvProblem& p, int rows, bool allow_ksplit, int n_cu) {
    const int nchunks = p.cin / SK, co_tiles = p.cout / 64;
    const long long pixels = (long long)p.height * p.width;
    PcChoice best{0, 32, 1, 1e30, 0, 0, 0};
    for (int shape = 1; shape <= 3; ++shape) {
        for (int tw : {32, 16, 8}) {
            if (shape == 1 && tw != 32) continue;
            const int th = kPcPix[shape] / tw;
            const long long tiles = (long long)ceil_div_i(p.width, tw) * ceil_div_i(rows, th) * co_tiles;
            for (int ks = 1; ks <= 16; ks *= 2) {
                if (ks > 1 && (!allow_ksplit || !p.scratch || shape == 1 || nchunks % ks != 0 || nchunks / ks < 2 ||
                               (size_t)ks * p.cout * pixels > kConvScratchFloats))
                    continue;
                const long long rounds = (tiles * ks + n_cu - 1) / n_cu;
                double cost = kPcLaunch + (double)rounds * ((double)(nchunks / ks) * kPcChunk[shape] + kPcRound[shape]);
                static Option reduce_pen("ST_CONV_PC_REDUCE_US", 4);
                static Option reduce_px("ST_CONV_PC_REDUCE_PIXELS", 4096);
                if (ks > 1)
                    cost += kPcReduce0 + ((pixels >= reduce_px.get() && nchunks >= 32) ? reduce_pen.get() : 0) +
                            kPcReduce1 * (double)ks * (double)p.cout * (double)pixels;
                if (cost < 0.97 * best.cost) best = PcChoice{shape, tw, ks, cost, 0, 0, 0};
            }
        }
    }
    return best;
}

// ... 27 lines not shown
    const int nchunks = p.cin / SK, co_tiles = p.cout / 64;
    PcChoice best = choose_pc_single(p, p.height, true, n_cu);
    static Option split_opt("ST_CONV_PC_SPLIT", 1);
    if (!split_opt.get()) return best;
    for (int shape = 1; shape <= 2; ++shape) {
        for (int tw : {32, 16, 8}) {
            if (shape == 1 && tw != 32) continue;
            const int th = kPcPix[shape] / tw;
            const int tiles_y = ceil_div_i(p.height, th);
            const long long per_row = (long long)ceil_div_i(p.width, tw) * co_tiles;
            const long long total = per_row * tiles_y;
            const long long full_rounds = total / n_cu;
            if (full_rounds < 1 || total % n_cu == 0) continue;
            const int rows_a = (int)((full_rounds * n_cu) / per_row);
            if (rows_a < 1 || rows_a >= tiles_y) continue;
            const long long rounds_a = (per_row * rows_a + n_cu - 1) / n_cu;
            const double cost_a = kPcLaunch + (double)rounds_a * ((double)nchunks * kPcChunk[shape] + kPcRound[shape]);
            const PcChoice rest = choose_pc_single(p, p.height - rows_a * th, false, n_cu);
            const double cost = cost_a + rest.cost;
            if (cost < 0.95 * best.cost) best = PcChoice{shape, tw, 1, cost, rows_a * th, rest.shape, rest.tw};
        }
    }
    return best;
}
}

namespace {
int pc_n_cu() {
    static int n_cu = 0;
    if (!n_cu) {
        int dev = 0;
        hipDeviceProp_t prop;
        n_cu = 256;
        if (hipGetDevice(&dev) == hipSuccess && hipGetDeviceProperties(&prop, dev) == hipSuccess && prop.multiProcessorCount >= 8)
            n_cu = prop.multiProcessorCount & ~7;
    }
    return n_cu;
}
}

bool conv_pc_fuses_pool(const ConvProblem& p) {
    static Option fuse_opt("ST_CONV_POOL_FUSE", 1);
    if (fuse_opt.get() && p.pool_out && !p.mask && !p.accumulate && !p.out_mask && conv_fat_preferred(p)) return true;
    static Option shape_opt("ST_CONV_PC_SHAPE", 0);
    static Option model_opt("ST_CONV_PC_MODEL", 1);
    static Option use_pc_opt("ST_CONV_PC", 1);
    if (!fuse_opt.get() || shape_opt.get() || !model_opt.get() || use_pc_opt.get() != 1) return false;
    if (!p.pool_out || p.mask || p.accumulate || p.out_mask || !conv_pc_applies(p)) return false;
    if (p.width % 4 != 0 || ((reinterpret_cast<uintptr_t>(p.out) | reinterpret_cast<uintptr_t>(p.pool_out)) & 15) != 0) return false;
    const PcChoice c = choose_pc_tile(p, pc_n_cu());
    auto ok = [](int shape, int tw) { return (shape == 1 || shape == 2) && tw == 32; };
    if (c.ksplit != 1 || !ok(c.shape, c.tw)) return false;
    return c.split_row == 0 || ok(c.shape2, c.tw2);
}

constexpr double kPcExchangeUs = 25.0;

bool conv_pc_overlap_choice(const ConvProblem& p_in, PcOverlap* out) {
    ConvProblem p = p_in;
    p.overlap_part = 0;
    p.row_begin = p.row_end = p.row_skip_begin = p.row_skip_len = 0;
    static Option mode_opt("ST_STRIP_OVERLAP", 1);
    static Option us_opt("ST_STRIP_OVERLAP_US", (int)kPcExchangeUs);
    static Option use_pc_opt("ST_CONV_PC", 1);
    ConvProblem q = p;
    if (!q.in_halo) q.in_halo = q.in;
    if (!use_pc_opt.get() || !mode_opt.get() || !conv_pc_applies(q) || !conv_pc_preferred(q)) return false;
    const int n_cu = pc_n_cu();
    const int nchunks = p.cin / SK, co_tiles = p.cout / 64;
    static Option fuse_opt("ST_CONV_POOL_FUSE", 1);
    static Option shape_opt("ST_CONV_PC_SHAPE", 0);
    static Option model_opt("ST_CONV_PC_MODEL", 1);
    const bool want_pool = fuse_opt.get() && !shape_opt.get() && model_opt.get() && use_pc_opt.get() == 1 &&
                           p.pool_out != nullptr && p.width % 4 == 0 && p.height % 2 == 0 && !p.mask && !p.accumulate && !p.out_mask &&
                           ((reinterpret_cast<uintptr_t>(p.out) | reinterpret_cast<uintptr_t>(p.pool_out)) & 15) == 0;
    auto pool_tile = [](int shape, int tw) { return (shape == 1 || shape == 2) && tw == 32; };
    struct Entry { int height, width, cin, cout, pool, scratch, n_cu; unsigned gen; bool valid; PcOverlap choice; };
    static Entry cache[64];
    static std::mutex guard;
    const unsigned gen = option_generation();
    const size_t slot = (size_t)(((unsigned long long)(unsigned)p.height * 0x9E3779B97F4A7C15ull ^
                                  (unsigned long long)(unsigned)p.width * 0xC2B2AE3D27D4EB4Full ^
                                  (unsigned long long)(unsigned)(p.cin * 1024 + p.cout) * 0x165667B19E3779F9ull ^ (unsigned)want_pool) >> 58);
    {
        std::lock_guard<std::mutex> lock(guard);
        const Entry& e = cache[slot];
        if (e.valid && e.gen == gen && e.height == p.height && e.width == p.width && e.cin == p.cin && e.cout == p.cout &&
            e.pool == (int)want_pool && e.scratch == (int)(p.scratch != nullptr) && e.n_cu == n_cu) {
            *out = e.choice;
            return true;
        }
    }
    PcOverlap best{};
    best.cost_split = 1e30;
    for (int shape_b = 1; shape_b <= 3; ++shape_b) {
        for (int tw_b : {32, 16, 8}) {
            if (shape_b == 1 && tw_b != 32) continue;
            if (want_pool && !pool_tile(shape_b, tw_b)) continue;
            const int th_b = kPcPix[shape_b] / tw_b;
            for (int k_bot = 1; k_bot <= 8; ++k_bot) {
                const int rows_b = (1 + k_bot) * th_b;
                if (p.height < rows_b + 2 || k_bot * th_b > p.height / 2) break;
                const long long tiles_b = (long long)ceil_div_i(p.width, tw_b) * (1 + k_bot) * co_tiles;
                const long long rounds_b = (tiles_b + n_cu - 1) / n_cu;
                const double cost_b = kPcLaunch + (double)rounds_b * ((double)nchunks * kPcChunk[shape_b] + kPcRound[shape_b]);
                PcChoice in_best{0, 32, 1, 1e30, 0, 0, 0};
// ... 123 lines not shown
```

style-transfer-pytorch_amd/csrc/st_conv_split.hip:

```cpp
#include <cstdlib>
#include <type_traits>

#include "st_common.h"

namespace st {
namespace {

typedef __bf16 bf16x8 __attribute__((ext_vector_type(8)));
typedef _Float16 f16x8 __attribute__((ext_vector_type(8)));
template <int E> struct Elem;
template <> struct Elem<0> { using scalar = __bf16; using vec = bf16x8; };
template <> struct Elem<1> { using scalar = _Float16; using vec = f16x8; };

__device__ __forceinline__ f32x16 mfma16(bf16x8 a, bf16x8 b, f32x16 c) {
    return __builtin_amdgcn_mfma_f32_32x32x16_bf16(a, b, c, 0, 0, 0);
}
__device__ __forceinline__ f32x16 mfma16(f16x8 a, f16x8 b, f32x16 c) {
    return __builtin_amdgcn_mfma_f32_32x32x16_f16(a, b, c, 0, 0, 0);
}

constexpr int SK = 16;
constexpr int kOOR = 0x40000000;

template <int B, int E, typename F>
// ... 473 lines not shown
    for (long long i = blockIdx.x * (long long)blockDim.x + threadIdx.x; i < total;
         i += (long long)gridDim.x * blockDim.x) {
        const int tap = (int)(i % 9);
        const int ci = (int)((i / 9) % cin);
        const int co = (int)(i / (9ll * cin));
        const int k = dgrad ? co : ci, m = dgrad ? ci : co, t = dgrad ? 8 - tap : tap;
        const size_t idx = (((size_t)t * (K / SK) + k / SK) * M + m) * SK + k % SK;
        float r = w[i] * scale;
        for (int pl = 0; pl < planes; ++pl) {
            const S h = (S)r;
            out[pl * plane + idx] = h;
            r = r - (float)h;
        }
    }
}

}

int launch_relayout_split(const float* w, void* out, int cin, int cout, int dgrad, int planes, int elem,
                          hipStream_t s) {
    ST_REQUIRE((planes == 2 || planes == 3) && (elem == 0 || (elem == 1 && planes == 2)),
               "split weights: planes %d / element type %d not supported", planes, elem);
    const size_t wcount = (size_t)cin * cout * 9;
    unsigned int* trailer = reinterpret_cast<unsigned int*>(static_cast<unsigned char*>(out) + wcount * 2 * planes);
    ST_HIP(hipMemsetAsync(trailer, 0, 256, s));
    if (launch_amax(w, (long long)wcount, trailer, 1, s)) return 1;
    if (elem == 1)
        hipLaunchKernelGGL(relayout_split_kernel<1>, dim3(1024), dim3(256), 0, s, w, static_cast<_Float16*>(out), cin,
                           cout, dgrad, planes);
    else
        hipLaunchKernelGGL(relayout_split_kernel<0>, dim3(1024), dim3(256), 0, s, w, static_cast<__bf16*>(out), cin,
                           cout, dgrad, planes);
    ST_LAUNCH_CHECK();
    return 0;
}

int fold_halo_amax(const ConvProblem& p, hipStream_t stream) {
    if (!p.in_halo || p.elem != 1 || !p.amax_word) return 0;
    const long long row = (long long)p.cin * p.width;
    if (p.has_up && p.has_down) return launch_amax(p.in_halo, 2 * row, p.amax_word, 0, stream);
    if (p.has_up) return launch_amax(p.in_halo, row, p.amax_word, 0, stream);
    if (p.has_down) return launch_amax(p.in_halo + (size_t)row, row, p.amax_word, 0, stream);
    return 0;
}

int launch_conv_split(const ConvProblem& p, hipStream_t stream) {
    ST_REQUIRE(p.taps == 9 && p.wgt_split != nullptr && (p.planes == 2 || p.planes == 3),
               "split conv: needs 3x3 taps and 2 or 3 weight planes");
    ST_REQUIRE(p.elem == 0 || (p.elem == 1 && p.planes == 2 && p.amax_word != nullptr),
               "split conv: fp16 planes need planes == 2 and an amax word");
    ST_REQUIRE(p.cin % SK == 0 && p.cout % 64 == 0, "split conv: Cin %% 16 and Cout %% 64 required (got %d, %d)",
               p.cin, p.cout);
    ST_REQUIRE((long long)p.height * p.width * SK * 4 < (1ll << 30), "split conv: image too large");
    const long long pixels = (long long)p.height * p.width;
    const int co_tiles = p.cout / 64;
    const long long wg_a = ((pixels + 255) / 256) * co_tiles, wg_b = ((pixels + 127) / 128) * co_tiles;
    const bool big = (wg_a >= 512) && p.planes != 3;
    long long wgs = big ? wg_a : wg_b;
    int ksplit = 1;
    if (p.scratch && !big) {
        const int nchunks = p.cin / SK;
        while (wgs * ksplit * 2 <= 640 && nchunks % (ksplit * 2) == 0 && nchunks / (ksplit * 2) >= 2 &&
               (size_t)(ksplit * 2) * p.cout * pixels <= kConvScratchFloats)
            ksplit *= 2;
    }
    if (p.elem == 1) {
        if (p.amax_measure && launch_amax(p.in, (long long)p.cin * pixels, p.amax_word, 0, stream)) return 1;
        if (!p.halo_amax_folded && fold_halo_amax(p, stream)) return 1;
        if (p.wgt_wino && p.wino && (p.wino > 1 ? conv_wino_applies(p) : conv_wino_preferred(p))) return launch_conv_wino(p, stream);
        if (conv_fat_preferred(p)) return launch_conv_fat(p, stream);
        static Option use_pc_opt("ST_CONV_PC", 1);
        const int use_pc = use_pc_opt.get();
        if (use_pc && (use_pc > 1 ? conv_pc_applies(p) : conv_pc_preferred(p))) return launch_conv_pc(p, stream);
        return big ? launch_split_tw<2, 2, 1>(p, ksplit, stream) : launch_split_tw<1, 2, 1>(p, ksplit, stream);
    }
    if (p.planes == 2) return big ? launch_split_tw<2, 2, 0>(p, ksplit, stream) : launch_split_tw<1, 2, 0>(p, ksplit, stream);
    return big ? launch_split_tw<2, 3, 0>(p, ksplit, stream) : launch_split_tw<1, 3, 0>(p, ksplit, stream);
}

}
```

style-transfer-pytorch_amd/csrc/st_conv_wino.hip:

```cpp
#include "st_common.h"

namespace st {
namespace {

typedef _Float16 f16x8 __attribute__((ext_vector_type(8)));
typedef _Float16 f16x4 __attribute__((ext_vector_type(4)));
typedef unsigned int u32x2 __attribute__((ext_vector_type(2)));

constexpr int kOOR = 0x40000000;
constexpr int kStage = 32768;
constexpr int kLdsA = 0, kLdsB = 2 * kStage;
constexpr int kLdsBytes = 4 * kStage;

template <int B, int E, typename F>
__device__ __forceinline__ void sfor(F&& f) {
    if constexpr (B < E) {
        f(std::integral_constant<int, B>{});
        sfor<B + 1, E>(f);
    }
}

__global__ __launch_bounds__(256) void wino_weights_kernel(const float* __restrict__ w, _Float16* __restrict__ out, int kdim, int mdim,
                                                          int dgrad, const unsigned int* __restrict__ w_amax, int* __restrict__ exp_out) {
    const int idx = blockIdx.x * 256 + threadIdx.x;
// ... 320 lines not shown
    for (int r = 0; r < 16; ++r)
        bias_r[r] = __builtin_bit_cast(float, __builtin_amdgcn_raw_buffer_load_b32(bs, (row0 + (r & 3) + 8 * (r >> 2)) * 4, 0, 0));
    unsigned int amax = 0;
    f32x2 nx_a0 = {0.f, 0.f}, nx_a1 = {0.f, 0.f}, nx_k0 = {0.f, 0.f}, nx_k1 = {0.f, 0.f};
    if constexpr (RMW) {
        nx_a0 = bload2(os_ld, off00, 0); nx_a1 = bload2(os_ld, off10, 0);
        nx_k0 = bload2(ms_ld, off00, 0); nx_k1 = bload2(ms_ld, off10, 0);
    }
    sfor<0, 16>([&](auto R) __attribute__((always_inline)) {
        constexpr int r = decltype(R)::value;
        constexpr int rr = (r & 3) + 8 * (r >> 2);
        const f32x2 a0 = nx_a0, a1 = nx_a1, k0 = nx_k0, k1 = nx_k1;
        if constexpr (RMW && r + 1 < 16) {
            constexpr int rn = ((r + 1) & 3) + 8 * ((r + 1) >> 2);
            const int n0 = in0 ? off00 + rn * hw4 : kOOR, n1 = in1 ? off10 + rn * hw4 : kOOR;
            nx_a0 = bload2(os_ld, n0, 0); nx_a1 = bload2(os_ld, n1, 0);
            nx_k0 = bload2(ms_ld, n0, 0); nx_k1 = bload2(ms_ld, n1, 0);
            __builtin_amdgcn_sched_barrier(0);
        }
        float s0[4], s1[4];
#pragma unroll
        for (int b = 0; b < 4; ++b) {
            s0[b] = (acc[0 + b][r] + acc[4 + b][r]) + acc[8 + b][r];
            s1[b] = (acc[4 + b][r] - acc[8 + b][r]) - acc[12 + b][r];
        }
        const float bias = bias_r[r];
        f32x2 y0v, y1v;
        y0v[0] = fmaxf(((s0[0] + s0[1]) + s0[2]) * unscale + bias, relu_floor);
        y0v[1] = fmaxf(((s0[1] - s0[2]) - s0[3]) * unscale + bias, relu_floor);
        y1v[0] = fmaxf(((s1[0] + s1[1]) + s1[2]) * unscale + bias, relu_floor);
        y1v[1] = fmaxf(((s1[1] - s1[2]) - s1[3]) * unscale + bias, relu_floor);
        if constexpr (RMW) {
            y0v += a0;
            y1v += a1;
            y0v[0] = k0[0] > mask_thr ? y0v[0] : 0.f; y0v[1] = k0[1] > mask_thr ? y0v[1] : 0.f;
            y1v[0] = k1[0] > mask_thr ? y1v[0] : 0.f; y1v[1] = k1[1] > mask_thr ? y1v[1] : 0.f;
        }
        amax = max(amax, in0 ? max(abs_bits(y0v[0]), abs_bits(y0v[1])) : 0u);
        amax = max(amax, in1 ? max(abs_bits(y1v[0]), abs_bits(y1v[1])) : 0u);
        const int o0 = in0 ? off00 + rr * hw4 : kOOR, o1 = in1 ? off10 + rr * hw4 : kOOR;
        if (RMW || !coded) {
            bstore2(y0v, os, o0);
            bstore2(y1v, os, o1);
        }
        if constexpr (!RMW) {
            if (pool) {
                float m = y0v[0];
                int at = 0;
                if (y0v[1] > m) { m = y0v[1]; at = 1; }
                if (y1v[0] > m) { m = y1v[0]; at = 2; }
                if (y1v[1] > m) { m = y1v[1]; at = 3; }
                const int po = in1 ? poff0 + rr * (PH * PW * 4) : kOOR;
                __builtin_amdgcn_raw_buffer_store_b32(__builtin_bit_cast(unsigned int, m), ps, po, 0, 0);
                __builtin_amdgcn_raw_buffer_store_b8((unsigned char)(at | (m > 0.f ? 4 : 0)), cs, in1 ? (po >> 2) : kOOR, 0, 0);
            }
        }
    });
    if (p.out_amax && !partial) amax_commit(amax, p.out_amax);
}

int wino_force_tx() {
    static Option tx_opt("ST_WINO_TX", 0);
    return tx_opt.get();
}

}

size_t winograd_weight_bytes(int cin, int cout) { return (size_t)16 * cin * cout * 2 * sizeof(_Float16) + 256; }

bool conv_wino_applies(const ConvProblem& p) {
    return p.taps == 9 && p.planes == 2 && p.elem == 1 && p.wgt_wino && p.amax_word && !p.mask && !p.in_halo && p.cin % 16 == 0 &&
           p.cout % 64 == 0 && p.width % 2 == 0 && p.width >= 2 && p.height >= 1 && p.row_begin == 0 && p.row_end == 0 &&
           p.row_skip_len == 0 && p.overlap_part == 0 && (long long)16 * p.height * p.width * 4 < (long long)kOOR &&
           (long long)p.height * p.width * 32 * 4 < (1ll << 31);
}

bool conv_wino_preferred(const ConvProblem& p) {
    static Option use_opt("ST_CONV_WINO", 1);
    return use_opt.get() != 0 && conv_wino_applies(p);
}

int launch_winograd_weights(const float* w, void* out, int cin, int cout, int dgrad, hipStream_t s) {
    unsigned int* trailer = reinterpret_cast<unsigned int*>(static_cast<unsigned char*>(out) + (size_t)16 * cin * cout * 2 * sizeof(_Float16));
    ST_HIP(hipMemsetAsync(trailer, 0, 256, s));
    if (launch_amax(w, (long long)cin * cout * 9, trailer, 1, s)) return 1;
    const int kdim = dgrad ? cout : cin, mdim = dgrad ? cin : cout;
    hipLaunchKernelGGL(wino_weights_kernel, dim3((cin * cout + 255) / 256), dim3(256), 0, s, w, static_cast<_Float16*>(out), kdim, mdim,
                       dgrad, trailer, reinterpret_cast<int*>(trailer + 8));
    ST_LAUNCH_CHECK();
    return 0;
}

namespace {
template <int TX, bool RMW, int TUNE = 0>
int launch_wino_cfg(const ConvProblem& p, int ksplit, hipStream_t s) {
    constexpr int TY = 64 / TX;
    auto kern = wino_conv_kernel<TX, RMW, TUNE>;
    static bool attr = false;
    if (!attr) {
        ST_HIP(hipFuncSetAttribute(reinterpret_cast<const void*>(kern), hipFuncAttributeMaxDynamicSharedMemorySize, kLdsBytes));
        attr = true;
    }
    const int tiles_x = ceil_div(p.width, 2 * TX), tiles_y = ceil_div(p.height, 2 * TY);
    const int n_co = p.cout / 64;
    const long long total = (long long)tiles_x * tiles_y * n_co * ksplit;
    ST_REQUIRE(total > 0 && total < (1ll << 30), "winograd conv: grid out of range");
    hipLaunchKernelGGL(kern, dim3((unsigned)total), dim3(256), kLdsBytes, s, p, tiles_x, n_co, ksplit, p.cin / 16 / ksplit, (int)total);
// ... 65 lines not shown
```

style-transfer-pytorch_amd/csrc/st_ops.hip:

```cpp
#include <cstdlib>
#include <vector>

#include "../../include/st_amd.h"
#include "st_common.h"

namespace st {
namespace {

struct OpScratch {
    hipStream_t stream;
    std::vector<void*> buffers;
    std::vector<hipEvent_t> events;
    explicit OpScratch(hipStream_t s) : stream(s) {}
    OpScratch(const OpScratch&) = delete;
    OpScratch& operator=(const OpScratch&) = delete;
    ~OpScratch() {
        hipStreamSynchronize(stream);
        for (void* b : buffers) hipFree(b);
        for (hipEvent_t e : events) hipEventDestroy(e);
    }
    template <class T>
    int alloc(T** out, size_t bytes) {
        void* p = nullptr;
        ST_HIP(hipMalloc(&p, bytes));
// ... 68 lines not shown
    OpScratch tmp(s);
    float *base = nullptr, *a = nullptr, *root = nullptr, *g = nullptr, *ga = nullptr, *gd = nullptr;
    if (tmp.alloc(&base, ns_workspace_floats(n) * 4) || tmp.alloc(&a, nn * 4) || tmp.alloc(&root, nn * 4) ||
        tmp.alloc(&g, nn * 4) || tmp.alloc(&ga, nn * 4) || tmp.alloc(&gd, 256))
        return 1;
    std::vector<float> h(nn, 0.f);
    unsigned x = 777u;
    for (size_t i = 0; i < nn; ++i) { x = x * 1664525u + 1013904223u; h[i] = ((int)(x >> 9) % 2001 - 1000) * 1e-4f; }
    for (int i = 0; i < n; ++i)
        for (int j = 0; j < i; ++j) h[(size_t)i * n + j] = h[(size_t)j * n + i];
    for (int i = 0; i < n; ++i) h[(size_t)i * n + i] = 1.0f + 0.1f * (i % 7);
    ST_HIP(hipMemcpy(a, h.data(), nn * 4, hipMemcpyHostToDevice));
    ST_HIP(hipMemcpy(g, h.data(), nn * 4, hipMemcpyHostToDevice));
    NSWorkspace ws{};
    ns_workspace_carve(ws, base, n);
    if (ns_workspace_reset(ws, s)) return 1;
    hipEvent_t e0, e1, e2;
    if (tmp.event(&e0) || tmp.event(&e1) || tmp.event(&e2)) return 1;
    static Option diag_opt("ST_NS_TIME_DIAG", 0);
    const bool diag = diag_opt.get() != 0;
    const float gdv = -2.f / n;
    ST_HIP(hipMemcpy(gd, &gdv, sizeof(float), hipMemcpyHostToDevice));
    const float* gfull = diag ? nullptr : g;
    const float* gdiag = diag ? gd : nullptr;
    if (ns_sqrt_forward(a, root, n, ws, s) || ns_sqrt_backward(root, gfull, gdiag, ga, n, ws, s)) return 1;
    ST_HIP(hipEventRecord(e0, s));
    for (int i = 0; i < iters; ++i)
        if (ns_sqrt_forward(a, root, n, ws, s)) return 1;
    ST_HIP(hipEventRecord(e1, s));
    for (int i = 0; i < iters; ++i)
        if (ns_sqrt_backward(root, gfull, gdiag, ga, n, ws, s)) return 1;
    ST_HIP(hipEventRecord(e2, s));
    ST_HIP(hipEventSynchronize(e2));
    float f = 0.f, b = 0.f;
    ST_HIP(hipEventElapsedTime(&f, e0, e1));
    ST_HIP(hipEventElapsedTime(&b, e1, e2));
    *fwd_us = f * 1e3 / iters;
    *bwd_us = b * 1e3 / iters;
    return ns_chain_check(ws, "st_op_sqrtm_time");
}

int st_op_tv_loss(const float* image, int height, int width, float* loss_out, float* grad_out, void* stream) {
    ST_REQUIRE(image && loss_out && grad_out, "st_op_tv_loss: null argument");
    hipStream_t s = static_cast<hipStream_t>(stream);
    OpScratch tmp(s);
    float* partials = nullptr;
    if (tmp.alloc(&partials, 4 * kStreamBlocks * sizeof(float))) return 1;
    return launch_tv(image, height, width, 1.0f, grad_out, partials, loss_out, s);
}

static int conv_op(const float* in, const float* mask, const float* weight, const float* bias, float* out,
                   int cin, int cout, int height, int width, int relu, int dgrad, int precision, hipStream_t s,
                   const float* halo = nullptr, int has_up = 0, int has_down = 0, int accumulate = 0,
                   const float* out_mask = nullptr, int overlap = 0) {
    if (reject_winograd(precision)) return 1;
    const bool wino5 = precision == 5;
    if (wino5) precision = 4;
    ST_REQUIRE(conv_precision_valid(precision), "conv precision must be 0, 2, 3 or 4");
    OpScratch tmp(s);
    float* wl = nullptr;
    float* scratch = nullptr;
    unsigned int* amax = nullptr;
    if (tmp.alloc(&wl, (size_t)cin * cout * 9 * sizeof(float)) || tmp.alloc(&scratch, kConvScratchFloats * sizeof(float)) ||
        tmp.alloc(&amax, kAmaxWordUints * 4))
        return 1;
    ST_HIP(hipMemsetAsync(amax, 0, kAmaxWordUints * 4, s));
    ConvProblem c{};
    c.scratch = scratch;
    if (precision > 0) {
        c.planes = conv_precision_planes(precision);
        c.elem = conv_precision_elem(precision);
        c.amax_word = amax;
        c.amax_measure = 1;
        void* wsplit = nullptr;
        if (tmp.alloc(&wsplit, split_weight_bytes(cin, cout, c.planes)) ||
            launch_relayout_split(weight, wsplit, cin, cout, dgrad, c.planes, c.elem, s))
            return 1;
        c.wgt_split = wsplit;
    }
    if (wino5) {
        void* wino = nullptr;
        if (tmp.alloc(&wino, winograd_weight_bytes(cin, cout)) || launch_winograd_weights(weight, wino, cin, cout, dgrad, s))
            return 1;
        c.wgt_wino = wino;
        c.wino = 2;
    }
    if (!dgrad) {
        if (launch_relayout_fwd(weight, wl, cin, cout, s)) return 1;
        c.cin = cin; c.cout = cout;
    } else {
        if (launch_relayout_dgrad(weight, wl, cin, cout, s)) return 1;
        c.cin = cout; c.cout = cin;
    }
    c.in = in; c.mask = mask; c.wgt = wl; c.bias = bias; c.out = out; c.height = height; c.width = width;
    c.taps = 9; c.relu = relu; c.accumulate = accumulate; c.out_mask = out_mask;
    c.in_halo = halo; c.has_up = halo ? has_up : 0; c.has_down = halo ? has_down : 0;
    if (overlap) {
        PcOverlap o{};
        ST_REQUIRE(conv_pc_overlap_choice(c, &o), "st_op_conv3x3_strip_ex: this problem cannot be cut into interior + boundary launches");
        ConvProblem part = c;
        part.overlap_part = 1; part.in_halo = nullptr; part.has_up = 0; part.has_down = 0;
        if (launch_conv(part, s)) return 1;
        part = c;
        part.overlap_part = 2; part.amax_measure = 0;
        return launch_conv(part, s);
    }
    return launch_conv(c, s);
}

int st_op_conv1x1(const float* in, const float* weight, const float* bias, float* out, int cin, int cout,
                  long long npix, int precision, void* stream) {
    ST_REQUIRE(in && weight && out, "st_op_conv1x1: null argument");
    ST_REQUIRE(precision == 0 || precision == 4, "st_op_conv1x1: precision must be 0 (fp32) or 4 (fp16x3)");
    ST_REQUIRE(cin % 32 == 0 && cout % 64 == 0 && npix > 0 && npix < (1ll << 31), "st_op_conv1x1: bad shape");
    hipStream_t s = static_cast<hipStream_t>(stream);
    OpScratch tmp(s);
    unsigned int* amax = nullptr;
    float* scratch = nullptr;
    if (tmp.alloc(&amax, 2 * kAmaxWordUints * 4) || tmp.alloc(&scratch, kConvScratchFloats * sizeof(float))) return 1;
    ST_HIP(hipMemsetAsync(amax, 0, 2 * kAmaxWordUints * 4, s));
    ConvProblem c{};
    c.in = in; c.wgt = weight; c.bias = bias; c.out = out; c.cin = cin; c.cout = cout;
    c.height = 1; c.width = (int)npix; c.taps = 1; c.scratch = scratch;
    if (precision == 4) {
        c.planes = 2; c.elem = 1; c.amax_word = amax; c.wgt_amax = amax + kAmaxWordUints;
        if (launch_amax(in, (long long)cin * npix, amax, 0, s) || launch_amax(weight, (long long)cin * cout, amax + kAmaxWordUints, 0, s))
            return 1;
    }
    return launch_conv(c, s);
}

int st_op_pool2x2(const float* in, float* out, int channels, int height, int width, int mode, void* stream) {
    ST_REQUIRE(in && out, "st_op_pool2x2: null argument");
    ST_REQUIRE(mode >= 0 && mode <= 2, "st_op_pool2x2: mode must be 0 (max), 1 (average) or 2 (l2)");
    ST_REQUIRE(channels > 0 && height >= 2 && width >= 2, "st_op_pool2x2: C >= 1 and H, W >= 2 required");
    return launch_pool_fwd(in, out, channels, height, width, mode, static_cast<hipStream_t>(stream));
}

int st_op_pool2x2_backward(const float* in, const float* grad_out, float* grad_in, int channels, int height, int width,
                           int mode, void* stream) {
    ST_REQUIRE(in && grad_out && grad_in, "st_op_pool2x2_backward: null argument");
    ST_REQUIRE(mode >= 0 && mode <= 2, "st_op_pool2x2_backward: mode must be 0 (max), 1 (average) or 2 (l2)");
    ST_REQUIRE(channels > 0 && height >= 2 && width >= 2, "st_op_pool2x2_backward: C >= 1 and H, W >= 2 required");
    return launch_pool_bwd(in, grad_out, grad_in, channels, height, width, mode, static_cast<hipStream_t>(stream));
}

int st_op_conv3x3_time(int cin, int cout, int height, int width, int dgrad, int precision, int iters,
                       double* avg_us, void* stream) {
    ST_REQUIRE(avg_us && iters > 0, "st_op_conv3x3_time: bad argument");
// ... 55 lines not shown
    if (tmp.event(&e0) || tmp.event(&e1)) return 1;
    ST_HIP(hipEventRecord(e0, s));
    for (int i = 0; i < iters; ++i)
        if (launch()) return 1;
    ST_HIP(hipEventRecord(e1, s));
    ST_HIP(hipEventSynchronize(e1));
    float ms = 0.f;
    ST_HIP(hipEventElapsedTime(&ms, e0, e1));
    *avg_us = ms * 1e3 / iters;
    if (option_env("ST_CONV_PHASES")) {
        const char* tune_env = option_env("ST_CONV_TUNE");
        const int keep = tune_env ? atoi(tune_env) : 0;
        c.tune = keep | 32;
        ST_HIP(hipMemsetAsync(scratch, 0, 1 << 20, s));
        for (int i = 0; i < 4; ++i)
            if (launch_conv(c, s)) return 1;
        ST_HIP(hipStreamSynchronize(s));
        c.tune = 0;
        {
            std::vector<unsigned long long> st(8 * 4096);
            ST_HIP(hipMemcpy(st.data(), scratch, st.size() * 8, hipMemcpyDeviceToHost));
            double ph[8] = {0, 0, 0, 0, 0, 0, 0, 0};
            int n = 0;
            for (int b = 0; b < 4096; ++b) {
                if (st[8 * b + 6] != 1) continue;
                for (int k = 0; k < 8; ++k) ph[k] += (double)st[8 * b + k];
                ++n;
            }
            if (n)
                fprintf(stderr, "[phases] %d->%d @%d dgrad %d tune %d: %d WGs, ticks avg per WG: consumer MFMA %.0f | consumer barrier "
                        "wait %.0f | epilogue %.0f | producer staging %.0f | producer barrier wait %.0f | whole %.0f; shader "
                        "clock %.0f MHz; %.1f us\n",
                        cin, cout, height, dgrad, keep, n, ph[0] / n, ph[1] / n, ph[2] / n, ph[3] / n, ph[4] / n, ph[5] / n,
                        ph[7] > 0 ? ph[5] / ph[7] * 100.0 : 0.0, *avg_us);
        }
    }
    return 0;
}

int st_op_conv3x3(const float* in, const float* weight, const float* bias, float* out, int cin, int cout,
                  int height, int width, int relu, int precision, void* stream) {
    ST_REQUIRE(in && weight && out, "st_op_conv3x3: null argument");
    return conv_op(in, nullptr, weight, bias, out, cin, cout, height, width, relu, 0, precision,
                   static_cast<hipStream_t>(stream));
}

int st_op_conv3x3_dgrad(const float* grad_out, const float* relu_out, const float* weight, float* grad_in,
                        int cin, int cout, int height, int width, int precision, void* stream) {
    ST_REQUIRE(grad_out && weight && grad_in, "st_op_conv3x3_dgrad: null argument");
    return conv_op(grad_out, relu_out, weight, nullptr, grad_in, cin, cout, height, width, 0, 1, precision,
                   static_cast<hipStream_t>(stream));
}

int st_op_conv3x3_strip(const float* in, const float* halo, int has_up, int has_down, const float* weight,
                        const float* bias, float* out, int cin, int cout, int height, int width, int relu, int dgrad,
                        int precision, void* stream) {
    ST_REQUIRE(in && halo && weight && out, "st_op_conv3x3_strip: null argument");
    return conv_op(in, nullptr, weight, dgrad ? nullptr : bias, out, cin, cout, height, width, dgrad ? 0 : relu, dgrad,
                   precision, static_cast<hipStream_t>(stream), halo, has_up != 0, has_down != 0);
}

int st_op_conv3x3_strip_ex(const float* in, const float* halo, int has_up, int has_down, const float* weight,
                           const float* bias, float* out, const float* out_mask, int cin, int cout, int height, int width,
                           int relu, int dgrad, int accumulate, int overlap, int precision, void* stream) {
    ST_REQUIRE(in && weight && out, "st_op_conv3x3_strip_ex: null argument");
    return conv_op(in, nullptr, weight, dgrad ? nullptr : bias, out, cin, cout, height, width, dgrad ? 0 : relu, dgrad,
                   precision, static_cast<hipStream_t>(stream), halo, has_up != 0, has_down != 0, accumulate != 0, out_mask,
                   overlap);
}

}
```

style-transfer-pytorch_amd/csrc/st_plan.h:

```cpp
#pragma once

#include <functional>
#include <unordered_map>
#include <vector>

#include "../../include/st_amd.h"
#include "st_common.h"
#include "st_head_core.h"

namespace st {

struct OpDesc {
    int kind;
    int index;
    int feat_index;
    int cin, cout;
};
const OpDesc kProgram[] = {
    {0, 0, 1, 3, 64},     {0, 1, 3, 64, 64},    {1, 0, 4, 64, 64},    {0, 2, 6, 64, 128},
    {0, 3, 8, 128, 128},  {1, 1, 9, 128, 128},  {0, 4, 11, 128, 256}, {0, 5, 13, 256, 256},
    {0, 6, 15, 256, 256}, {0, 7, 17, 256, 256}, {1, 2, 18, 256, 256}, {0, 8, 20, 256, 512},
    {0, 9, 22, 512, 512}, {0, 10, 24, 512, 512}, {0, 11, 26, 512, 512}, {1, 3, 27, 512, 512},
    {0, 12, 29, 512, 512},
};
constexpr int kNumOps = sizeof(kProgram) / sizeof(kProgram[0]);
constexpr float kCovEps = 1e-4f;

struct Node {
    float* y = nullptr;
    float* g = nullptr;
    float* yhalo = nullptr;
    float* ghalo = nullptr;
    int c = 0, h = 0, w = 0;
    int hg = 0;
    bool pooled_by_conv = false;
    unsigned char* pool_code = nullptr;
    bool coded = false;
    unsigned int* y_amax = nullptr;
    unsigned int* g_amax = nullptr;
    size_t count() const { return (size_t)c * h * w; }
};

struct HeadSite {
    StyleHead* h = nullptr;
    const Node* tap = nullptr;
    float weight = 0.f;
    float eps = kCovEps;
    float* loss = nullptr;
    float* grad = nullptr;
    unsigned int* grad_amax = nullptr;
    int slot = -1;
    const float* sqrt_mask = nullptr;
    float mask_sum = 0.f;
};

struct ProfileEvent {
    hipEvent_t start, stop;
    double flops;
};

enum HbmCat { HBM_CONV1_FWD = 0, HBM_CONV1_DGRAD, HBM_POOL_BWD, HBM_ADAM, HBM_TV, HBM_GRAM1, HBM_CONTENT, HBM_HEAD_1X1, HBM_CATS };
struct HbmEvent {
    hipEvent_t start, stop;
    int cat;
    double bytes;
};

}

struct st_net {
    int pooling = 0;
    float* w_first = nullptr;
    float w_first_l1max = 0.f;
    float b_first_max = 0.f;
    float* bias[13] = {};
    float* w_fwd[13] = {};
    float* w_bwd[13] = {};
    int conv_planes = 0;
    int conv_elem = 0;
    void* ws_fwd[13] = {};
    void* ws_bwd[13] = {};
    int wide_fwd[13] = {};
    int wide_bwd[13] = {};
    void* wsx_fwd[13] = {};
    void* wsx_bwd[13] = {};
    float* w_torch[13] = {};
    int guard_fwd[13] = {};
    int guard_bwd[13] = {};
};

// ... 58 lines not shown
    float* lossbuf = nullptr;
    float* gram_raw[5] = {};
    long long gram_total = 0;
    hipStream_t comm_stream = nullptr;
    bool comm_stream_borrowed = false;
    hipStream_t chain_stream = nullptr;
    hipEvent_t moments_ready[5] = {}, chain_done[5] = {};
    hipEvent_t pack_done = nullptr, halo_landed = nullptr;
    unsigned int* halo_bound = nullptr;

    int rank = 0, world = 1;
    float* head_result[5] = {};
    struct Phase {
        std::function<int(hipStream_t)> run;
        st_exchange ex;
        const float* halo = nullptr;
    };
    std::unordered_map<const float*, bool> halo_inline;
    std::vector<Phase> phases;
    size_t phase_pos = 0;
    const float* ph_image = nullptr;
    float* ph_grad = nullptr;
    int ph_last_layer = -1;
    unsigned ph_option_gen = 0;
    hipStream_t head_stream[5] = {};
    bool head_stream_owned[5] = {};
    hipEvent_t tap_ready[5] = {};
    hipEvent_t head_done[5] = {};
    bool streams_ready = false;
    int device = 0;
    bool graph_enabled = false;
    hipStream_t main_stream = nullptr;
    bool gram1_fused = false;
    int gram1_splits = 0;
    bool compact_streams = false;
    bool head4_on_caller = false;
    std::vector<hipStream_t> junk_streams;
    hipEvent_t bridge_in = nullptr, bridge_out = nullptr;
    hipStream_t aux_stream = nullptr;
    hipEvent_t aux_in = nullptr, aux_fwd = nullptr, tv_done = nullptr, content_done = nullptr;
    hipGraph_t graph = nullptr;
    hipGraphExec_t graph_exec = nullptr;
    const float* gk_image = nullptr;
    float* gk_grad = nullptr;
    float* gk_losses = nullptr;
    int gk_seen = 0;
    bool capturing = false;
    bool timeline = false;
    hipEvent_t tl_start = nullptr, tl_fwd = nullptr, tl_head[5] = {}, tl_bwd = nullptr;
    hipEvent_t tl_h4[4] = {};
    hipEvent_t tl_h3[4] = {};
    int tl_count = 0;
    bool profiling = false;
    std::vector<st::ProfileEvent> events;
    size_t events_used = 0;
    std::vector<st::HbmEvent> hbm_events;
    size_t hbm_used = 0;
    long long prof_launches = 0;
    double prof_ms = 0, prof_flops = 0;
    bool defer_sum = false;
    bool amax_clean = false;
    const st::FoldUpdate* fold_update = nullptr;
    bool fold_updated = false;
};

namespace st {

inline Node& node_at(st_plan* p, int op) { return kProgram[op].kind == 0 ? p->conv[kProgram[op].index] : p->pool[kProgram[op].index]; }
inline const Node& node_at(const st_plan* p, int op) { return node_at(const_cast<st_plan*>(p), op); }
inline bool head_taps_conv(const st_plan* p, int k, int conv_index) {
    return kProgram[p->style_op[k]].kind == 0 && kProgram[p->style_op[k]].index == conv_index;
}
inline void assign_head_bounds(st_plan* p) {
    unsigned int* words = reinterpret_cast<unsigned int*>(p->amax_word);
    for (StyleHead& h : p->head) h.s_amax = words + (size_t)63 * kAmaxWordUints;
    for (int j = 0; j < p->n_style; ++j) p->head[p->style_op[j]].s_amax = words + (size_t)(48 + j) * kAmaxWordUints;
    for (int r = 1; r < kMaxRegions; ++r) {
        for (StyleHead& h : p->region_head[r - 1]) h.s_amax = nullptr;
        for (int j = 0; p->region_amax && j < p->n_style; ++j)
            p->region_head[r - 1][p->style_op[j]].s_amax = p->region_amax + (size_t)((r - 1) * 16 + j) * kAmaxWordUints;
    }
}
inline StyleHead& region_head_at(st_plan* p, int region, int op) { return region == 0 ? p->head[op] : p->region_head[region - 1][op]; }
inline const StyleHead& region_head_at(const st_plan* p, int region, int op) { return region_head_at(const_cast<st_plan*>(p), region, op); }

constexpr int kHaloTrailer = 16;

int plan_alloc(st_plan* p, float** out, size_t floats);
struct PlanAlloc { st_plan* p; int operator()(float** out, size_t floats) const { return *out ? 0 : plan_alloc(p, out, floats); } };
int conv_launch_profiled(st_plan* p, const ConvProblem& prob, hipStream_t s, double flops_fraction = 1.0);
template <class F>
int hbm_profiled(st_plan* p, int cat, double bytes, hipStream_t s, F&& launch) {
    if (!p->profiling) return launch();
    if (p->hbm_used == p->hbm_events.size()) {
        HbmEvent ev{};
        ST_HIP(hipEventCreate(&ev.start));
        ST_HIP(hipEventCreate(&ev.stop));
        p->hbm_events.push_back(ev);
    }
    HbmEvent& ev = p->hbm_events[p->hbm_used++];
    ev.cat = cat;
    ev.bytes = bytes;
    ST_HIP(hipEventRecord(ev.start, s));
    const int rc = launch();
    ST_HIP(hipEventRecord(ev.stop, s));
    return rc;
// ... 43 lines not shown
```

style-transfer-pytorch_amd/csrc/st_pool.hip:

```cpp
#include "st_common.h"

namespace st {
namespace {

constexpr float kAvgScale = 2.0f;
constexpr float kL2Scale = 0.78f;

__global__ __launch_bounds__(256) void pool_fwd_kernel(const float* __restrict__ in, float* __restrict__ out,
                                                       int C, int H, int W, int mode) {
#pragma clang fp contract(off)
    const int Ho = H / 2, Wo = W / 2;
    const long long total = (long long)C * Ho * Wo;
    for (long long i = blockIdx.x * 256ll + threadIdx.x; i < total; i += (long long)gridDim.x * 256) {
        const int xo = (int)(i % Wo);
        const int yo = (int)((i / Wo) % Ho);
        const int c = (int)(i / ((long long)Wo * Ho));
        const float* p = in + ((size_t)c * H + 2 * yo) * W + 2 * xo;
        const float a = p[0], b = p[1], d = p[W], e = p[W + 1];
        float r;
        if (mode == 0) {
            r = a;
            if (b > r) r = b;
            if (d > r) r = d;
            if (e > r) r = e;
// ... 74 lines not shown
        o[1] = pool_window(r0[2], r0[3], r1[2], r1[3], mode);
        *reinterpret_cast<f32x2*>(out + (size_t)row * (W / 2) + 2 * x4) = o;
    }
}

__device__ __forceinline__ void pool_window_bwd(float a, float b, float d, float e, float go, int mode, float& ga,
                                                float& gb, float& gd, float& ge) {
#pragma clang fp contract(off)
    if (mode == 0) {
        int arg = 0;
        float m = a;
        if (b > m) { m = b; arg = 1; }
        if (d > m) { m = d; arg = 2; }
        if (e > m) { m = e; arg = 3; }
        ga = arg == 0 ? go : 0.f; gb = arg == 1 ? go : 0.f; gd = arg == 2 ? go : 0.f; ge = arg == 3 ? go : 0.f;
    } else if (mode == 1) {
        ga = gb = gd = ge = (go * kAvgScale) / 4.f;
    } else {
        const float m = (a * a + b * b + d * d + e * e) / 4.f;
        const float root = sqrtf(m * 4.f);
        const float s = go * kL2Scale;
        ga = s * (a / root); gb = s * (b / root); gd = s * (d / root); ge = s * (e / root);
    }
    ga = a > 0.f ? ga : 0.f; gb = b > 0.f ? gb : 0.f; gd = d > 0.f ? gd : 0.f; ge = e > 0.f ? ge : 0.f;
}

__global__ __launch_bounds__(256) void pool_bwd4_kernel(const float* __restrict__ in,
                                                        const float* __restrict__ gout, float* __restrict__ gin,
                                                        int C, int H, int W, int mode) {
    const int Ho = H / 2, W4 = W / 4;
    const long long total = (long long)C * Ho * W4;
    for (long long i = blockIdx.x * 256ll + threadIdx.x; i < total; i += (long long)gridDim.x * 256) {
        const int x4 = (int)(i % W4);
        const long long row = i / W4;
        const int yo = (int)(row % Ho);
        const long long c = row / Ho;
        const size_t base = ((size_t)c * H + 2 * yo) * W + 4 * x4;
        const f32x4 r0 = *reinterpret_cast<const f32x4*>(in + base), r1 = *reinterpret_cast<const f32x4*>(in + base + W);
        const f32x2 go = *reinterpret_cast<const f32x2*>(gout + (size_t)row * (W / 2) + 2 * x4);
        f32x4 g0, g1;
        float ga, gb, gd, ge;
        pool_window_bwd(r0[0], r0[1], r1[0], r1[1], go[0], mode, ga, gb, gd, ge);
        g0[0] = ga; g0[1] = gb; g1[0] = gd; g1[1] = ge;
        pool_window_bwd(r0[2], r0[3], r1[2], r1[3], go[1], mode, ga, gb, gd, ge);
        g0[2] = ga; g0[3] = gb; g1[2] = gd; g1[3] = ge;
        *reinterpret_cast<f32x4*>(gin + base) = g0;
        *reinterpret_cast<f32x4*>(gin + base + W) = g1;
    }
}

__global__ __launch_bounds__(256) void pool_bwd_codes_kernel(const unsigned char* __restrict__ code,
                                                             const float* __restrict__ gout, float* __restrict__ gin,
                                                             int C, int H, int W) {
    const int Ho = H / 2, W4 = W / 4;
    const long long total = (long long)C * Ho * W4;
    for (long long i = blockIdx.x * 256ll + threadIdx.x; i < total; i += (long long)gridDim.x * 256) {
        const int x4 = (int)(i % W4);
        const long long row = i / W4;
        const int yo = (int)(row % Ho);
        const long long c = row / Ho;
        const size_t base = ((size_t)c * H + 2 * yo) * W + 4 * x4;
        const size_t pooled = (size_t)row * (W / 2) + 2 * x4;
        const unsigned short two = *reinterpret_cast<const unsigned short*>(code + pooled);
        const f32x2 go = *reinterpret_cast<const f32x2*>(gout + pooled);
        f32x4 g0 = {0.f, 0.f, 0.f, 0.f}, g1 = {0.f, 0.f, 0.f, 0.f};
#pragma unroll
        for (int w = 0; w < 2; ++w) {
            const int cd = (two >> (8 * w)) & 0xff;
            const float g = (cd & 4) ? go[w] : 0.f;
            const int at = cd & 3;
            g0[2 * w] = at == 0 ? g : 0.f;
            g0[2 * w + 1] = at == 1 ? g : 0.f;
            g1[2 * w] = at == 2 ? g : 0.f;
            g1[2 * w + 1] = at == 3 ? g : 0.f;
        }
        *reinterpret_cast<f32x4*>(gin + base) = g0;
        *reinterpret_cast<f32x4*>(gin + base + W) = g1;
    }
}

}

int launch_pool_bwd_codes(const unsigned char* code, const float* grad_out, float* grad_in, int channels, int height,
                          int width, hipStream_t s) {
    ST_REQUIRE(width % 4 == 0 && height % 2 == 0, "pool backward from codes: W %% 4 == 0 and even H required");
    const long long total4 = (long long)channels * (height / 2) * (width / 4);
    const int blocks4 = (int)std::min<long long>((total4 + 255) / 256, 16384);
    hipLaunchKernelGGL(pool_bwd_codes_kernel, dim3(blocks4), dim3(256), 0, s, code, grad_out, grad_in, channels, height, width);
    ST_LAUNCH_CHECK();
    return 0;
}

int launch_pool_fwd(const float* in, float* out, int channels, int height, int width, int mode,
                    hipStream_t s) {
    const bool aligned = ((reinterpret_cast<uintptr_t>(in) | reinterpret_cast<uintptr_t>(out)) & 15) == 0;
    if (width % 4 == 0 && aligned) {
        const long long total4 = (long long)channels * (height / 2) * (width / 4);
        const int blocks4 = (int)std::min<long long>((total4 + 255) / 256, 16384);
        hipLaunchKernelGGL(pool_fwd4_kernel, dim3(blocks4), dim3(256), 0, s, in, out, channels, height, width, mode);
        ST_LAUNCH_CHECK();
        return 0;
    }
    const long long total = (long long)channels * (height / 2) * (width / 2);
    const int blocks = (int)std::min<long long>((total + 255) / 256, 8192);
    hipLaunchKernelGGL(pool_fwd_kernel, dim3(blocks), dim3(256), 0, s, in, out, channels, height, width, mode);
    ST_LAUNCH_CHECK();
    return 0;
}

int launch_pool_bwd(const float* in, const float* grad_out, float* grad_in, int channels, int height,
                    int width, int mode, hipStream_t s) {
    const bool aligned = ((reinterpret_cast<uintptr_t>(in) | reinterpret_cast<uintptr_t>(grad_out) |
                           reinterpret_cast<uintptr_t>(grad_in)) & 15) == 0;
    if (width % 4 == 0 && height % 2 == 0 && aligned) {
        const long long total4 = (long long)channels * (height / 2) * (width / 4);
        const int blocks4 = (int)std::min<long long>((total4 + 255) / 256, 16384);
        hipLaunchKernelGGL(pool_bwd4_kernel, dim3(blocks4), dim3(256), 0, s, in, grad_out, grad_in, channels, height,
                           width, mode);
        ST_LAUNCH_CHECK();
        return 0;
    }
    const long long total = (long long)channels * height * width;
    const int blocks = (int)std::min<long long>((total + 255) / 256, 8192);
    hipLaunchKernelGGL(pool_bwd_kernel, dim3(blocks), dim3(256), 0, s, in, grad_out, grad_in, channels,
                       height, width, mode);
    ST_LAUNCH_CHECK();
    return 0;
}

}
```

style-transfer-pytorch_amd/style_transfer/_hip.py:

```python

import ctypes
import os

import torch

_PKG_ROOT = os.path.dirname(os.path.dirname(os.path.abspath(__file__)))
_LIB_CANDIDATES = (os.path.join(_PKG_ROOT, 'lib', 'libst_amd.so'),
                   os.path.join(os.path.dirname(os.path.abspath(__file__)), 'lib', 'libst_amd.so'))
LIB_PATH = next((c for c in _LIB_CANDIDATES if os.path.exists(c)), _LIB_CANDIDATES[0])

_c_float_p = ctypes.c_void_p
TAPS = (1, 3, 4, 6, 8, 9, 11, 13, 15, 17, 18, 20, 22, 24, 26, 27, 29)
DEFAULT_CONTENT_LAYERS, DEFAULT_STYLE_LAYERS = (22,), (1, 6, 11, 20, 29)
CONTENT_LOSSES, STYLE_LOSSES = ('mse', 'scaled_mse'), ('w2', 'gram')
_lib = None


class HipLibraryError(RuntimeError):
    pass


class Exchange(ctypes.Structure):
    _fields_ = [('kind', ctypes.c_int), ('count', ctypes.c_longlong), ('send_up', ctypes.c_void_p),
                ('send_down', ctypes.c_void_p), ('recv_up', ctypes.c_void_p), ('recv_down', ctypes.c_void_p),
# ... 27 lines not shown
        'st_plan_moments': (i32, [vp, i32, vp, vp, vp]),
        'st_plan_set_style_mask': (i32, [vp, vp, vp]),
        'st_plan_style_mask': (i32, [vp, i32, pp, ip, ip, ctypes.POINTER(f64)]),
        'st_plan_set_style_regions': (i32, [vp, i32, pp, vp]),
        'st_plan_style_region': (i32, [vp, i32, i32, pp, ip, ip, ctypes.POINTER(f64)]),
        'st_plan_set_region_style_target': (i32, [vp, i32, i32, vp, vp, vp]),
        'st_plan_set_region_weights': (i32, [vp, ctypes.POINTER(f32)]),
        'st_plan_region_terms': (i32, [vp, pp, ip, ip]),
        'st_plan_set_content_mask': (i32, [vp, vp, vp]),
        'st_plan_content_mask': (i32, [vp, i32, pp, ip, ip]),
        'st_plan_set_tv_mask': (i32, [vp, vp, vp]),
        'st_plan_tv_mask': (i32, [vp, pp, ip, ip]),
        'st_plan_set_content_target': (i32, [vp, vp, vp]),
        'st_plan_set_style_target': (i32, [vp, i32, vp, vp, vp]),
        'st_plan_set_loss_weights': (i32, [vp, f32, ctypes.POINTER(f32), f32]),
        'st_plan_set_taps': (i32, [vp, i32, ip, i32, ip]),
        'st_plan_set_tap_weights': (i32, [vp, ctypes.POINTER(f32), ctypes.POINTER(f32), f32]),
        'st_plan_set_loss_kinds': (i32, [vp, i32, i32]),
        'st_plan_loss_kinds': (i32, [vp, ip, ip]),
        'st_plan_set_layer_loss_kinds': (i32, [vp, ip, ip]),
        'st_plan_layer_loss_kinds': (i32, [vp, ip, ip]),
        'st_plan_set_loss_eps': (i32, [vp, ctypes.POINTER(f32), ctypes.POINTER(f32)]),
        'st_plan_loss_eps': (i32, [vp, ctypes.POINTER(f32), ctypes.POINTER(f32)]),
        'st_plan_set_content_target_at': (i32, [vp, i32, vp, vp]),
        'st_plan_term_losses': (i32, [vp, pp, ip]),
        'st_plan_loss_and_grad': (i32, [vp, vp, vp, vp, vp]),
        'st_plan_step': (i32, [vp, vp, vp, vp, vp, i64, f64, f64, f64, f64, f64, vp, vp]),
        'st_plan_apply_update': (i32, [vp, vp, vp, vp, vp, vp, i64, f64, f64, f64, f64, f64, vp]),
        'st_lbfgs_state_bytes': (i64, [i64]),
        'st_lbfgs_reset': (i32, [vp, i64, vp]),
        'st_lbfgs_update': (i32, [vp, i64, vp, vp, vp, f64, vp]),
        'st_plan_lbfgs_step': (i32, [vp, vp, vp, vp, f64, vp, vp]),
        'st_lbfgs_info': (i32, [vp, i64, ip, ip, ip, ip, ctypes.POINTER(f64), ctypes.POINTER(f64), vp]),
        'st_qn_strip_state_bytes': (i64, [i64, i32]),
        'st_qn_strip_dots': (i32, [vp, i64, i32, i32, vp, ctypes.POINTER(Exchange), vp]),
        'st_qn_strip_apply': (i32, [vp, i64, i32, vp, vp, vp, f64, vp]),
        'st_plan_qn_strip_step': (i32, [vp, vp, vp, vp, vp, vp, f64, vp]),
        'st_plan_create_strip': (i32, [pp, vp, i32, i32, i32, i32]),
        'st_plan_closure_begin': (i32, [vp, vp, vp]),
        'st_plan_set_rank': (i32, [vp, i32, i32]),
        'st_plan_closure_next': (i32, [vp, ctypes.POINTER(Exchange), vp]),
        'st_fabric_unique_id': (i32, [ctypes.c_char_p]),
        'st_fabric_create': (i32, [pp, ctypes.c_char_p, ctypes.c_char_p, i32, i32, i32]),
        'st_fabric_destroy': (i32, [vp]),
        'st_fabric_abort': (i32, [vp]),
        'st_fabric_selftest': (i32, [vp, vp, i32]),
        'st_plan_closure_run': (i32, [vp, vp, vp]),
        'st_plan_losses': (i32, [vp, pp]),
        'st_plan_debug_read': (i32, [vp, i32, ctypes.POINTER(f32), i32]),
        'st_plan_forward_begin': (i32, [vp, vp, i32]),
        'st_plan_moment_sums': (i32, [vp, i32, vp, vp]),
        'st_plan_set_graph': (i32, [vp, i32]),
        'st_plan_profile_enable': (i32, [vp, i32]),
        'st_plan_profile_read': (i32, [vp, ctypes.POINTER(i64), ctypes.POINTER(f64), ctypes.POINTER(f64)]),
        'st_plan_profile_read_hbm': (i32, [vp, i32, ctypes.POINTER(i64), ctypes.POINTER(f64), ctypes.POINTER(f64)]),
        'st_op_sqrtm_ns': (i32, [vp, vp, i32, vp]),
        'st_op_sqrtm_ns_backward': (i32, [vp, vp, vp, i32, vp]),
        'st_op_sqrtm_ns_backward_diag': (i32, [vp, f32, vp, i32, vp]),
        'st_op_tv_loss': (i32, [vp, i32, i32, vp, vp, vp]),
        'st_op_sqrtm_time': (i32, [i32, i32, ctypes.POINTER(f64), ctypes.POINTER(f64), vp]),
        'st_op_mfma_rate': (i32, [i32, i32, i32, i32, ctypes.POINTER(f64), ctypes.POINTER(f64), vp]),
        'st_op_mfma_valu_rate': (i32, [i32, i32, i32, i32, i32, i32, i32, ctypes.POINTER(f64), ctypes.POINTER(f64),
                                       ctypes.POINTER(f64), vp]),
        'st_op_grid_barrier_time': (i32, [i32, i32, i32, i32, ctypes.POINTER(f64), ip, vp]),
        'st_op_winograd_consumer_rate': (i32, [i32, i32, ctypes.POINTER(f64), vp]),
        'st_op_conv3x3_time': (i32, [i32, i32, i32, i32, i32, i32, i32, ctypes.POINTER(f64), vp]),
        'st_op_conv3x3': (i32, [vp, vp, vp, vp, i32, i32, i32, i32, i32, i32, vp]),
        'st_op_conv3x3_dgrad': (i32, [vp, vp, vp, vp, i32, i32, i32, i32, i32, vp]),
        'st_op_conv3x3_strip': (i32, [vp, vp, i32, i32, vp, vp, vp, i32, i32, i32, i32, i32, i32, i32, vp]),
        'st_op_conv3x3_strip_ex': (i32, [vp, vp, i32, i32, vp, vp, vp, vp, i32, i32, i32, i32, i32, i32, i32, i32, i32, vp]),
        'st_op_conv1x1': (i32, [vp, vp, vp, vp, i32, i32, i64, i32, vp]),
        'st_op_pool2x2': (i32, [vp, vp, i32, i32, i32, i32, vp]),
        'st_op_pool2x2_backward': (i32, [vp, vp, vp, i32, i32, i32, i32, vp]),
        'st_head_create': (i32, [pp, i32, i32, i32, i32, i32]),
        'st_head_destroy': (i32, [vp]),
        'st_head_device_bytes': (i64, [vp]),
        'st_head_state_floats': (i64, [vp]),
        'st_head_moments': (i32, [vp, vp, vp, vp, vp]),
        'st_head_forward': (i32, [vp, vp, vp, vp, vp, vp, f32, vp, vp, vp]),
        'st_head_backward': (i32, [vp, vp, vp, vp, vp, vp]),
        'st_op_reduce_scratch_floats': (i64, []),
        'st_op_mse_loss': (i32, [vp, vp, i64, vp, vp, vp]),
        'st_op_mse_loss_backward': (i32, [vp, vp, i64, vp, vp, vp]),
        'st_op_scaled_mse_loss': (i32, [vp, vp, i64, f32, vp, vp, vp, vp]),
        'st_op_scaled_mse_loss_backward': (i32, [vp, vp, i64, vp, vp, vp, vp]),
        'st_op_tv_value': (i32, [vp, i32, i32, vp, vp, vp]),
        'st_op_tv_loss_backward': (i32, [vp, i32, i32, vp, vp, vp]),
    }
    for name, (res, args) in sig.items():
        fn = getattr(lib, name)
        fn.restype = res
        fn.argtypes = args
    return sig


EXPORTED_SYMBOLS = None


def load_library(require_gpu=True):
    global _lib, EXPORTED_SYMBOLS
    if _lib is None:
        if not os.path.exists(LIB_PATH):
            raise HipLibraryError(
                f'{LIB_PATH} not found: build it with `python style-transfer-pytorch_amd/build.py` '
                '(needs hipcc, targets gfx950).  This package has no CPU or PyTorch fallback.')
        lib = ctypes.CDLL(LIB_PATH)
        EXPORTED_SYMBOLS = sorted(_declare(lib))
        if lib.st_abi_version() != 2:
            raise HipLibraryError('libst_amd.so ABI version mismatch')
        _lib = lib
    if require_gpu and not torch.cuda.is_available():
        raise HipLibraryError('no HIP device visible: the MI355X hot path cannot run (no CPU fallback)')
    return _lib


def has_experiments():
    return bool(load_library(require_gpu=False).st_has_experiments())


def env_switches():
    lib = load_library(require_gpu=False)
# ... 372 lines not shown
        with torch.cuda.device(self.device):
            _check(self.lib.st_plan_set_style_target(self.handle, int(index), _ptr(mean.contiguous()),
                                                     _ptr(srm.contiguous()), _stream()))

    def set_loss_weights(self, content_weight, style_layer_weights, tv_weight):
        nc, ns = len(self.content_layers), len(self.style_layers)
        try:
            cws = [float(w) for w in content_weight]
        except TypeError:
            cws = [float(content_weight)] * nc
        sws = [float(w) for w in style_layer_weights]
        if (tuple(self.content_layers), tuple(self.style_layers)) == (DEFAULT_CONTENT_LAYERS, DEFAULT_STYLE_LAYERS):
            sws += [0.0] * (ns - len(sws))
        if len(cws) != nc or len(sws) != ns:
            raise ValueError(f'{len(cws)} content and {len(sws)} style weights for {nc} content and {ns} style layers')
        ca, sa = (ctypes.c_float * max(nc, 1))(*cws), (ctypes.c_float * max(ns, 1))(*sws)
        _check(self.lib.st_plan_set_tap_weights(self.handle, ca, sa, float(tv_weight)))

    def loss_and_grad(self, image, grad_out=None):
        if grad_out is None:
            grad_out = torch.empty_like(image)
        self.forward_count += 1
        with torch.cuda.device(self.device):
            _check(self.lib.st_plan_loss_and_grad(self.handle, self._img(image), _ptr(grad_out),
                                                  _ptr(self.losses), _stream()))
        return self.losses, grad_out

    def step(self, image, exp_avg, exp_avg_sq, ema_value, step, lr, beta1=0.9, beta2=0.99, eps=1e-8,
             ema_decay=0.99):
        self.forward_count += 1
        with torch.cuda.device(self.device):
            _check(self.lib.st_plan_step(self.handle, self._img(image), _ptr(exp_avg), _ptr(exp_avg_sq),
                                         _ptr(ema_value), int(step), float(lr), float(beta1), float(beta2),
                                         float(eps), float(ema_decay), _ptr(self.losses), _stream()))
        return self.losses

    def apply_update(self, image, grad, exp_avg, exp_avg_sq, ema_value, step, lr, beta1=0.9, beta2=0.99, eps=1e-8,
                     ema_decay=0.99):
        with torch.cuda.device(self.device):
            _check(self.lib.st_plan_apply_update(self.handle, self._img(image), _ptr(grad), _ptr(exp_avg), _ptr(exp_avg_sq),
                                                 _ptr(ema_value), int(step), float(lr), float(beta1), float(beta2),
                                                 float(eps), float(ema_decay), _stream()))

    def range_guard(self, image):
        fwd, bwd = (ctypes.c_int * 13)(), (ctypes.c_int * 13)()
        self.forward_count += 1
        with torch.cuda.device(self.device):
            _check(self.lib.st_plan_range_guard(self.handle, self._img(image), fwd, bwd, _stream()))
        return list(fwd), list(bwd)

    def set_graph(self, on=True):
        _check(self.lib.st_plan_set_graph(self.handle, 1 if on else 0))

    def profile_enable(self, on=True):
        _check(self.lib.st_plan_profile_enable(self.handle, 1 if on else 0))

    HBM_KERNELS = ('conv1_1 forward (+ normalize)', 'conv1_1 data gradient (+ pad fold)', 'max-pool backward (4 levels)',
                   'Adam + clamp + EMA', 'TV loss + gradient', 'relu1_1 Gram + mean', 'content MSE + gradient',
                   "style heads' 1x1 gradient step (5 taps)")

    def profile_read_hbm(self):
        out = {}
        for cat, name in enumerate(self.HBM_KERNELS):
            n, ms, by = ctypes.c_longlong(), ctypes.c_double(), ctypes.c_double()
            _check(self.lib.st_plan_profile_read_hbm(self.handle, cat, ctypes.byref(n), ctypes.byref(ms), ctypes.byref(by)))
            out[name] = (n.value, ms.value, by.value)
        return out

    def profile_read(self):
        n, ms, fl = ctypes.c_longlong(), ctypes.c_double(), ctypes.c_double()
        _check(self.lib.st_plan_profile_read(self.handle, ctypes.byref(n), ctypes.byref(ms), ctypes.byref(fl)))
        return n.value, ms.value, fl.value


class LBFGS:

    EXITS = ('moved', 'gradient', 'change')

    def __init__(self, like, rank=0, world=1):
        self.lib = load_library()
        self.device = like.device
        self.count = like.numel()
        self.rank, self.world = int(rank), int(world)
        nbytes = int(self.lib.st_qn_strip_state_bytes(self.count, self.world))
        if nbytes <= 0 or not 0 <= self.rank < self.world:
            raise ValueError(f'LBFGS: rank {rank} of {world} ranks (1 ... 8) for {self.count} elements')
        self._exchange = Exchange()
        self.state = torch.empty((nbytes + 3) // 4, device=self.device, dtype=torch.float32)
        self.reset()

    def _state(self):
        return ctypes.c_void_p(self.state.data_ptr())

    def reset(self):
        with torch.cuda.device(self.device):
            _check(self.lib.st_lbfgs_reset(self._state(), self.count, _stream()))

    def step(self, plan, image, ema_value, ema_decay):
        assert image.numel() == self.count
        plan.forward_count += 1
        with torch.cuda.device(self.device):
            _check(self.lib.st_plan_lbfgs_step(plan.handle, plan._img(image), self._state(), _ptr(ema_value),
                                               float(ema_decay), _ptr(plan.losses), _stream()))
        return plan.losses

    def update(self, image, grad, ema_value=None, ema_decay=0.99):
# ... 257 lines not shown

def op_conv1x1(x, weight, bias, precision=0):
    lib = load_library()
    cout, cin = weight.shape
    npix = x.shape[1]
    out = torch.empty((cout, npix), device=x.device, dtype=torch.float32)
    with torch.cuda.device(x.device):
        _check(lib.st_op_conv1x1(_ptr(x.contiguous()), _ptr(weight.contiguous()),
                                 _ptr(bias.contiguous()) if bias is not None else None, _ptr(out), cin, cout,
                                 npix, int(precision), _stream()))
    return out


POOL_MODES = {'max': 0, 'average': 1, 'l2': 2}


def op_pool2x2(x, pooling, out=None):
    lib = load_library()
    c, h, w = x.shape[-3:]
    if out is None:
        out = torch.empty((c, h // 2, w // 2), device=x.device, dtype=torch.float32)
    assert out.numel() == c * (h // 2) * (w // 2)
    with torch.cuda.device(x.device):
        _check(lib.st_op_pool2x2(_ptr(x.contiguous()), _ptr(out), c, h, w, POOL_MODES[pooling], _stream()))
    return out


def op_pool2x2_backward(x, grad_out, pooling, grad_in=None):
    lib = load_library()
    c, h, w = x.shape[-3:]
    assert grad_out.numel() == c * (h // 2) * (w // 2)
    if grad_in is None:
        grad_in = torch.empty((c, h, w), device=x.device, dtype=torch.float32)
    assert grad_in.numel() == c * h * w
    with torch.cuda.device(x.device):
        _check(lib.st_op_pool2x2_backward(_ptr(x.contiguous()), _ptr(grad_out.contiguous()), _ptr(grad_in), c, h, w,
                                          POOL_MODES[pooling], _stream()))
    return grad_in


def op_conv3x3_dgrad(grad_out, relu_out, weight, precision=0):
    lib = load_library()
    cout, cin = weight.shape[:2]
    h, w = grad_out.shape[-2:]
    gin = torch.empty((1, cin, h, w), device=grad_out.device, dtype=torch.float32)
    with torch.cuda.device(grad_out.device):
        _check(lib.st_op_conv3x3_dgrad(_ptr(grad_out.contiguous()),
                                       _ptr(relu_out.contiguous()) if relu_out is not None else None,
                                       _ptr(weight.contiguous()), _ptr(gin), cin, cout, h, w, int(precision),
                                       _stream()))
    return gin


def _reduce_scratch(device):
    return torch.empty(int(load_library().st_op_reduce_scratch_floats()), device=device, dtype=torch.float32)


def op_mse_loss(x, target):
    lib = load_library()
    loss = torch.empty((), device=x.device, dtype=torch.float32)
    with torch.cuda.device(x.device):
        _check(lib.st_op_mse_loss(_ptr(x), _ptr(target), x.numel(), _ptr(_reduce_scratch(x.device)), _ptr(loss), _stream()))
    return loss


def op_mse_loss_backward(x, target, upstream):
    lib = load_library()
    grad = torch.empty(x.shape, device=x.device, dtype=torch.float32)
    with torch.cuda.device(x.device):
        _check(lib.st_op_mse_loss_backward(_ptr(x), _ptr(target), x.numel(), _ptr(upstream), _ptr(grad), _stream()))
    return grad


def op_scaled_mse_loss(x, target, eps):
    lib = load_library()
    loss = torch.empty((), device=x.device, dtype=torch.float32)
    totals = torch.empty(2, device=x.device, dtype=torch.float32)
    with torch.cuda.device(x.device):
        _check(lib.st_op_scaled_mse_loss(_ptr(x), _ptr(target), x.numel(), float(eps), _ptr(_reduce_scratch(x.device)),
                                         _ptr(totals), _ptr(loss), _stream()))
    return loss, totals


def op_scaled_mse_loss_backward(x, target, totals, upstream):
    lib = load_library()
    grad = torch.empty(x.shape, device=x.device, dtype=torch.float32)
    with torch.cuda.device(x.device):
        _check(lib.st_op_scaled_mse_loss_backward(_ptr(x), _ptr(target), x.numel(), _ptr(totals), _ptr(upstream), _ptr(grad),
                                                  _stream()))
    return grad


def op_tv_value(image):
    lib = load_library()
    h, w = image.shape[-2:]
    loss = torch.empty((), device=image.device, dtype=torch.float32)
    with torch.cuda.device(image.device):
        _check(lib.st_op_tv_value(_ptr(image), h, w, _ptr(_reduce_scratch(image.device)), _ptr(loss), _stream()))
    return loss


def op_tv_loss_backward(image, upstream):
    lib = load_library()
    h, w = image.shape[-2:]
    grad = torch.empty(image.shape, device=image.device, dtype=torch.float32)
    with torch.cuda.device(image.device):
# ... 3 lines not shown
```

Before: 435.2 it/s.

## Fold max-pool backward into the following conv data-gradient producer stage

The backward pass no longer launches a separate max-pool backward kernel before the 3x3 data-gradient conv that consumes its output. Instead the conv's producer warps read the pooled gradient and the argmax codes directly and scatter them on the fly while staging into LDS. To make this possible, the pool codes are stored in a new channel-grouped byte layout (8 channels per window), and the standalone code-based pool backward kernel is rewritten to match. This removes a full-resolution gradient write plus read at each pooled level. The cost is extra code loads and masking in the producer, and a lazy fallback for debug reads.

```diff
diff --git a/include/st_amd.h b/include/st_amd.h
--- a/include/st_amd.h
+++ b/include/st_amd.h
@@ -146,6 +146,8 @@
                   int height, int width, int relu, int precision, void* stream);
 int st_op_conv3x3_dgrad(const float* grad_out, const float* relu_out, const float* weight, float* grad_in,
                         int cin, int cout, int height, int width, int precision, void* stream);
+int st_op_conv3x3_dgrad_pooled(const float* grad_pooled, const unsigned char* codes, const float* weight, float* grad_in,
+                               const float* out_mask, int cin, int cout, int height, int width, int accumulate, void* stream);
 int st_op_conv3x3_strip(const float* in, const float* halo, int has_up, int has_down, const float* weight,
                         const float* bias, float* out, int cin, int cout, int height, int width, int relu, int dgrad,
                         int precision, void* stream);
@@ -159,6 +161,8 @@
 int st_op_pool2x2(const float* in, float* out, int channels, int height, int width, int mode, void* stream);
 int st_op_pool2x2_backward(const float* in, const float* grad_out, float* grad_in, int channels, int height, int width,
                            int mode, void* stream);
+int st_op_pool2x2_backward_codes(const unsigned char* codes, const float* grad_out, float* grad_in, int channels, int height,
+                                 int width, void* stream);
 
 
 typedef struct st_head st_head;
@@ -198,6 +202,8 @@
 
 int st_plan_debug_read(st_plan* plan, int what, float* out, int count);
 
+int st_plan_pool_backward_counts(st_plan* plan, long long* launched, long long* folded);
+
 int st_op_grid_barrier_time(int workgroups, int rounds, int payload_floats, int groups, double* us_per_round, int* errors,
                             void* stream);
 
diff --git a/style-transfer-pytorch_amd/csrc/st_api.hip b/style-transfer-pytorch_amd/csrc/st_api.hip
--- a/style-transfer-pytorch_amd/csrc/st_api.hip
+++ b/style-transfer-pytorch_amd/csrc/st_api.hip
@@ -543,10 +543,24 @@
         return 0;
     }
     if (grad_map) {
+        if (kProgram[what - 16].kind == 0 && node_at(p, what - 16).g_folded) {
+            Node& cn = node_at(p, what - 16);
+            const Node& pn = node_at(p, what - 16 + 1);
+            if (launch_pool_bwd_codes(cn.pool_code, pn.g, cn.g, cn.c, cn.h, cn.w, nullptr)) return 1;
+            ST_HIP(hipDeviceSynchronize());
+            cn.g_folded = false;
+        }
         ST_HIP(hipMemcpy(out, node_at(p, what - 16).g, (size_t)count * sizeof(float), hipMemcpyDeviceToHost));
         return 0;
     }
     ST_HIP(hipMemcpy(out, what == 0 ? p->red_partials : tv_debug_buffer(), (size_t)count * sizeof(float), hipMemcpyDeviceToHost));
+    return 0;
+}
+
+int st_plan_pool_backward_counts(st_plan* p, long long* launched, long long* folded) {
+    ST_REQUIRE(p && launched && folded, "st_plan_pool_backward_counts: null argument");
+    *launched = p->pool_bwd_launched;
+    *folded = p->pool_bwd_folded;
     return 0;
 }
 
diff --git a/style-transfer-pytorch_amd/csrc/st_closure.hip b/style-transfer-pytorch_amd/csrc/st_closure.hip
--- a/style-transfer-pytorch_amd/csrc/st_closure.hip
+++ b/style-transfer-pytorch_amd/csrc/st_closure.hip
@@ -524,8 +524,24 @@
     c.amax_word = n.g_amax; c.out_amax = net->conv_elem == 1 ? in.g_amax : nullptr;
 }
 
+bool pool_bwd_fused(const st_plan* p, int i, ConvProblem& c) {
+    static Option fused_opt("ST_POOL_BWD_FUSED", 1);
+    const OpDesc& op = kProgram[i];
+    if (!fused_opt.get() || p->profiling || op.kind != 1 || i < 2 || kProgram[i - 1].kind != 0 || p->net->pooling != 0) return false;
+    const Node& in = p->conv[kProgram[i - 1].index];
+    if (!in.coded || !in.pool_code) return false;
+    dgrad_conv(p, i - 1, c);
+    if (c.mask) return false;
+    const Node& n = p->pool[op.index];
+    c.in = n.g;
+    c.in_pool_code = in.pool_code;
+    c.amax_word = n.g_amax;
+    return conv_pooled_input_applies(c);
+}
+
 int run_backward(st_plan* p, float* grad_image, hipStream_t s) {
     const st_net* net = p->net;
+    bool pool_folded = false;
     for (int i = kNumOps - 1; i >= 0; --i) {
         const OpDesc& op = kProgram[i];
         if (op.kind == 0) {
@@ -545,12 +561,27 @@
             if (pop.kind == 0 && join_head_for_conv(p, pop.index, s)) return 1;
             if (i - 1 == p->content_op[0]) ST_HIP(hipStreamWaitEvent(s, p->content_done, 0));
             ConvProblem c{};
-            dgrad_conv(p, i, c);
+            if (pool_folded) {
+                pool_folded = false;
+                ST_REQUIRE(pool_bwd_fused(p, i + 1, c), "closure: the pooled-input data gradient no longer applies");
+            } else {
+                dgrad_conv(p, i, c);
+            }
             if (conv_launch_profiled(p, c, s)) return 1;
         } else {
             Node& n = p->pool[op.index];
             const OpDesc& pop = kProgram[i - 1];
             Node& in = p->conv[pop.index];
+            {
+                ConvProblem c{};
+                pool_folded = pool_bwd_fused(p, i, c);
+                in.g_folded = pool_folded;
+                if (pool_folded) {
+                    ++p->pool_bwd_folded;
+                    continue;
+                }
+            }
+            ++p->pool_bwd_launched;
             const double bytes = in.coded ? (in.count() + 1.25 * n.count()) * 4.0 : (2.0 * in.count() + n.count()) * 4.0;
             if (hbm_profiled(p, HBM_POOL_BWD, bytes, s, [&] {
                     if (in.coded) return launch_pool_bwd_codes(in.pool_code, n.g, in.g, in.c, in.h, in.w, s);
@@ -601,6 +632,8 @@
             if (conv_launch_profiled(p, c, s)) return 1;
         } else {
             Node& n = p->pool[op.index];
+            in.g_folded = false;
+            ++p->pool_bwd_launched;
             if (hbm_profiled(p, HBM_POOL_BWD, (2.0 * in.count() + n.count()) * 4.0, s, [&] {
                     return launch_pool_bwd(in.y, n.g, in.g, in.c, in.h, in.w, net->pooling, s);
                 }))
diff --git a/style-transfer-pytorch_amd/csrc/st_common.h b/style-transfer-pytorch_amd/csrc/st_common.h
--- a/style-transfer-pytorch_amd/csrc/st_common.h
+++ b/style-transfer-pytorch_amd/csrc/st_common.h
@@ -147,6 +147,7 @@
     int overlap_part;
     float* pool_out;
     unsigned char* pool_code;
+    const unsigned char* in_pool_code;
     const void* wgt_wino;
     int wino;
 };
@@ -211,6 +212,7 @@
 int launch_amax(const float* x, long long n, unsigned int* word, int single, hipStream_t s);
 bool conv_pc_applies(const ConvProblem& p);
 bool conv_pc_preferred(const ConvProblem& p);
+bool conv_pooled_input_applies(const ConvProblem& p);
 int launch_conv_pc(const ConvProblem& p, hipStream_t stream);
 bool conv_fat_applies(const ConvProblem& p);
 bool conv_fat_preferred(const ConvProblem& p);
diff --git a/style-transfer-pytorch_amd/csrc/st_conv.hip b/style-transfer-pytorch_amd/csrc/st_conv.hip
--- a/style-transfer-pytorch_amd/csrc/st_conv.hip
+++ b/style-transfer-pytorch_amd/csrc/st_conv.hip
@@ -434,6 +434,7 @@
     ST_REQUIRE(p.taps == 9 || p.taps == 1, "conv: taps must be 9 or 1");
     if (p.planes > 0 && p.taps == 9 && p.wgt_split && p.cin % 16 == 0)
         return launch_conv_split(p, stream);
+    ST_REQUIRE(!p.in_pool_code, "conv: the pooled-input staging exists in the fp16x3 producer / consumer kernel only");
     const int KC = (p.taps == 9) ? kChunk3x3 : kChunk1x1;
     ST_REQUIRE(p.cin % KC == 0 && p.cout % 64 == 0, "conv: Cin %% %d and Cout %% 64 required (got %d, %d)", KC,
                p.cin, p.cout);
diff --git a/style-transfer-pytorch_amd/csrc/st_conv_fat.hip b/style-transfer-pytorch_amd/csrc/st_conv_fat.hip
--- a/style-transfer-pytorch_amd/csrc/st_conv_fat.hip
+++ b/style-transfer-pytorch_amd/csrc/st_conv_fat.hip
@@ -327,8 +327,10 @@
                     const unsigned poff = poff0 + (unsigned)q * pstep;
                     const f32x2 pv = {m0, m1};
                     __builtin_amdgcn_raw_buffer_store_b64(__builtin_bit_cast(u32x2, pv), ps, (int)poff, 0, 0);
-                    const int two = (at0 | (m0 > 0.f ? 4 : 0)) | ((at1 | (m1 > 0.f ? 4 : 0)) << 8);
-                    __builtin_amdgcn_raw_buffer_store_b16((unsigned short)two, cs, pin ? (int)(poff >> 2) : 0x7FFFFFFF, 0, 0);
+                    const unsigned cwin = pin ? (unsigned)((y >> 1) * PW + (x >> 1)) * 8u : 0x7FFFFFF0u;
+                    const unsigned coff = cwin + (unsigned)(q >> 2) * (unsigned)(PH * PW * 8) + (unsigned)(2 * (q & 3) + lrow);
+                    __builtin_amdgcn_raw_buffer_store_b8((unsigned char)(at0 | (m0 > 0.f ? 4 : 0)), cs, (int)coff, 0, 0);
+                    __builtin_amdgcn_raw_buffer_store_b8((unsigned char)(at1 | (m1 > 0.f ? 4 : 0)), cs, (int)(coff + 8u), 0, 0);
                 }
             }
             amax_e = max(amax_e, inb ? max(max(abs_bits(v[0]), abs_bits(v[1])), max(abs_bits(v[2]), abs_bits(v[3]))) : 0u);
diff --git a/style-transfer-pytorch_amd/csrc/st_conv_pc.hip b/style-transfer-pytorch_amd/csrc/st_conv_pc.hip
--- a/style-transfer-pytorch_amd/csrc/st_conv_pc.hip
+++ b/style-transfer-pytorch_amd/csrc/st_conv_pc.hip
@@ -59,9 +59,10 @@
     static constexpr int NWT = (NWP + PT - 1) / PT;
 };
 
-template <int TW, int WN, int CW, bool HALO>
+template <int TW, int WN, int CW, bool HALO, bool POOLED = false>
 __global__ __launch_bounds__((CW == 8 || WN == 1 ? 768 : 512), 1) void conv_pc_kernel(ConvProblem p, int tiles_x, int n_co_tiles, int ksplit,
                                                          int nchunks, int total) {
+    static_assert(!(HALO && POOLED), "the pooled-input staging has no halo rows");
     using C = PCfg<TW, WN, CW>;
     extern __shared__ __attribute__((aligned(16))) unsigned char smem[];
     const int tid = threadIdx.x, lane = tid & 63;
@@ -72,6 +73,7 @@
     const int ptid = tid - 64 * CW;
     const int l31 = lane & 31, half = lane >> 5;
     const int H = p.height, W = p.width, HW = H * W;
+    const int IW = POOLED ? W >> 1 : W, IHW = POOLED ? (H >> 1) * (W >> 1) : HW;
     const int Y0 = p.row_begin, Y1 = p.row_end ? p.row_end : H;
 
     const int my_tiles = (total - (int)blockIdx.x + (int)gridDim.x - 1) / (int)gridDim.x;
@@ -140,8 +142,13 @@
                 const int g = it / C::NPX, q = it % C::NPX;
                 const int y = t.y0 - 1 + q / C::LW, x = t.x0 - 1 + q % C::LW;
                 const bool ok = y >= 0 && y < H && x >= 0 && x < W;
+                if constexpr (POOLED) {
+                    goff[i] = ok ? (8 * g * IHW + (y >> 1) * IW + (x >> 1)) * 4 : kOOR;
+                    aoff[i] = q * 32 + ((g ^ ((q >> 3) & 1)) * 16) + (g << 2) + ((y & 1) << 1) + (x & 1);
+                } else {
                 goff[i] = ok ? (8 * g * HW + y * W + x) * 4 : kOOR;
                 aoff[i] = q * 32 + ((g ^ ((q >> 3) & 1)) * 16);
+                }
                 if constexpr (HALO) {
                     const bool xin = x >= 0 && x < W;
                     const bool top = xin && y == -1 && p.has_up, bot = xin && y == H && p.has_down;
@@ -153,8 +160,10 @@
         };
         float ract[C::SETS][C::NIT][8];
         float rhal[HALO ? C::SETS : 1][HALO ? C::NIT : 1][8];
+        typedef unsigned int u32x2 __attribute__((ext_vector_type(2)));
+        u32x2 rcode[POOLED ? C::SETS : 1][POOLED ? C::NIT : 1];
         f32x4 rwt[C::SETS][2][C::NWT];
-        const int chunk_bytes = SK * HW * 4;
+        const int chunk_bytes = SK * IHW * 4;
         int loaded = 0;
         constexpr int NA = C::NIT / 2;
         const bool ablate_prod = (p.tune & 256) != 0;
@@ -163,14 +172,25 @@
             constexpr int st = decltype(SET)::value, part = decltype(PART)::value;
             constexpr bool withw = decltype(WITHW)::value;
             if (ablate_prod || ablate_loads) return;
-            const int cc = l_chunk0 + l_chunk;
+            int cc = l_chunk0 + l_chunk;
+            if constexpr (POOLED) cc = __builtin_amdgcn_readfirstlane(cc);
             const __amdgpu_buffer_rsrc_t rs = __builtin_amdgcn_make_buffer_rsrc(
-                const_cast<float*>(p.in) + (size_t)cc * SK * HW, 0, chunk_bytes, 0x00020000);
+                const_cast<float*>(p.in) + (size_t)cc * SK * IHW, 0, chunk_bytes, 0x00020000);
             sfor<(part == 1 ? NA : 0), (part == 0 ? NA : C::NIT)>([&](auto I) __attribute__((always_inline)) {
                 constexpr int i = decltype(I)::value;
 #pragma unroll
-                for (int c = 0; c < 8; ++c) ract[st][i][c] = bload(rs, goff[i], c * HW * 4);
+                for (int c = 0; c < 8; ++c) ract[st][i][c] = bload(rs, goff[i], c * IHW * 4);
             });
+            if constexpr (POOLED) {
+                const __amdgpu_buffer_rsrc_t cs = __builtin_amdgcn_make_buffer_rsrc(
+                    const_cast<unsigned char*>(p.in_pool_code) + (size_t)cc * SK * IHW, 0, SK * IHW, 0x00020000);
+                const unsigned gsub = 56u * (unsigned)IHW;
+                sfor<(part == 1 ? NA : 0), (part == 0 ? NA : C::NIT)>([&](auto I) __attribute__((always_inline)) {
+                    constexpr int i = decltype(I)::value;
+                    const unsigned coff = 2u * (unsigned)goff[i] - ((aoff[i] & 4) ? gsub : 0u);
+                    rcode[st][i] = __builtin_bit_cast(u32x2, __builtin_amdgcn_raw_buffer_load_b64(cs, (int)coff, 0, 0));
+                });
+            }
             if constexpr (HALO) {
                 if constexpr (part != 1) set_halo[st][0] = halo_tile;
                 if constexpr (part != 0) set_halo[st][1] = halo_tile;
@@ -219,9 +239,12 @@
             sfor<(part == 1 ? NA : 0), (part == 0 ? NA : C::NIT)>([&](auto I) __attribute__((always_inline)) {
                 constexpr int i = decltype(I)::value;
                 f16x8 h0, h1;
+                u32x2 miss = {0u, 0u};
+                if constexpr (POOLED) miss = (rcode[st][i] & 0x07070707u) ^ ((4u | ((unsigned)aoff[i] & 3u)) * 0x01010101u);
 #pragma unroll
                 for (int c = 0; c < 8; ++c) {
                     float v = ract[st][i][c];
+                    if constexpr (POOLED) v = ((miss[c >> 2] >> (8 * (c & 3))) & 0xffu) == 0u ? v : 0.f;
                     if constexpr (HALO) {
                         if (set_halo[st][i < NA ? 0 : 1]) v += rhal[st][i][c];
                     }
@@ -230,8 +253,9 @@
                     h0[c] = a;
                     h1[c] = (_Float16)(v - (float)a);
                 }
-                *reinterpret_cast<f16x8*>(buf + aoff[i]) = h0;
-                *reinterpret_cast<f16x8*>(buf + C::ACT_PLANE + aoff[i]) = h1;
+                const int lds_at = POOLED ? (aoff[i] & ~15) : aoff[i];
+                *reinterpret_cast<f16x8*>(buf + lds_at) = h0;
+                *reinterpret_cast<f16x8*>(buf + C::ACT_PLANE + lds_at) = h1;
             });
             sfor<(part == 1 ? 1 : 0), (!withw ? 0 : part == 0 ? 1 : 2)>([&](auto PL) __attribute__((always_inline)) {
                 constexpr int pl = decltype(PL)::value;
@@ -545,8 +569,11 @@
                             __builtin_amdgcn_raw_buffer_store_b64(
                                 __builtin_bit_cast(__attribute__((__vector_size__(2 * sizeof(unsigned int)))) unsigned int, pv), ps, (int)poff, 0, 0);
                             if (coded) {
-                                const int two = (at0 | (m0 > 0.f ? 4 : 0)) | ((at1 | (m1 > 0.f ? 4 : 0)) << 8);
-                                __builtin_amdgcn_raw_buffer_store_b16((unsigned short)two, cs, pin ? (int)(poff >> 2) : 0x7FFFFFFF, 0, 0);
+                                const unsigned ch = (unsigned)(q4 * RG) + lrow;
+                                const unsigned win = pin ? (unsigned)((y >> 1) * PW + (x >> 1)) * 8u : 0x7FFFFFF0u;
+                                const unsigned coff = win + (ch >> 3) * (unsigned)(PH * PW * 8) + (ch & 7u);
+                                __builtin_amdgcn_raw_buffer_store_b8((unsigned char)(at0 | (m0 > 0.f ? 4 : 0)), cs, (int)coff, 0, 0);
+                                __builtin_amdgcn_raw_buffer_store_b8((unsigned char)(at1 | (m1 > 0.f ? 4 : 0)), cs, (int)(coff + 8u), 0, 0);
                             }
                         }
                     }
@@ -614,7 +641,7 @@
 
 inline int ceil_div_i(int a, int b) { return (a + b - 1) / b; }
 
-template <int TW, int WN, int CW, bool HALO>
+template <int TW, int WN, int CW, bool HALO, bool POOLED = false>
 int launch_pc_cfg_h(const ConvProblem& p, int ksplit, hipStream_t stream) {
     using C = PCfg<TW, WN, CW>;
     constexpr int LDS = 2 * C::BUF + (C::XL ? CW * 64 : CW * (32 * (WN * 32 + 8) + 64)) * 4;
@@ -622,7 +649,7 @@
     static_assert(LDS <= 160 * 1024, "LDS budget of one CU");
     static bool attr_set = false;
     static int n_cu = 256;
-    auto kern = conv_pc_kernel<TW, WN, CW, HALO>;
+    auto kern = conv_pc_kernel<TW, WN, CW, HALO, POOLED>;
     if (!attr_set) {
         ST_HIP(hipFuncSetAttribute(reinterpret_cast<const void*>(kern), hipFuncAttributeMaxDynamicSharedMemorySize, LDS));
         int dev = 0;
@@ -672,6 +699,12 @@
 
 template <int TW, int WN, int CW>
 int launch_pc_cfg(const ConvProblem& p, int ksplit, hipStream_t stream) {
+    if (p.in_pool_code) {
+        ST_REQUIRE(!p.in_halo && !p.mask && p.height % 2 == 0 && p.width % 4 == 0 && p.row_begin % 2 == 0 && p.row_skip_len == 0 &&
+                       p.overlap_part == 0,
+                   "conv (producer/consumer): pooled input needs even H, W %% 4 == 0, an even first row and no halo, mask or row cut");
+        return launch_pc_cfg_h<TW, WN, CW, false, true>(p, ksplit, stream);
+    }
     if (p.in_halo) return launch_pc_cfg_h<TW, WN, CW, true>(p, ksplit, stream);
     return launch_pc_cfg_h<TW, WN, CW, false>(p, ksplit, stream);
 }
@@ -692,6 +725,7 @@
 }
 
 namespace {
+constexpr int kPooledShapesDefault = 3;
 bool xl_tile_pays(const ConvProblem& p) {
     static Option xl_opt("ST_CONV_PC_XL", 1);
     const int xl = xl_opt.get();
@@ -825,6 +859,30 @@
     auto ok = [](int shape, int tw) { return (shape == 1 || shape == 2) && tw == 32; };
     if (c.ksplit != 1 || !ok(c.shape, c.tw)) return false;
     return c.split_row == 0 || ok(c.shape2, c.tw2);
+}
+
+bool conv_pooled_input_applies(const ConvProblem& p) {
+    static Option shapes_opt("ST_POOL_BWD_FUSED_SHAPES", kPooledShapesDefault);
+    static Option use_pc_opt("ST_CONV_PC", 1);
+    static Option shape_opt("ST_CONV_PC_SHAPE", 0);
+    static Option model_opt("ST_CONV_PC_MODEL", 1);
+    if (!p.in_pool_code || p.in_halo || p.mask || p.overlap_part != 0 || p.row_begin != 0 || p.row_end != 0 || p.row_skip_len != 0 ||
+        p.height % 2 != 0 || p.width % 4 != 0 || !conv_pc_applies(p))
+        return false;
+    if (p.wgt_wino && p.wino && (p.wino > 1 ? conv_wino_applies(p) : conv_wino_preferred(p))) return false;
+    if (conv_fat_preferred(p)) return false;
+    const int use_pc = use_pc_opt.get();
+    if (!use_pc || (use_pc == 1 && !conv_pc_preferred(p))) return false;
+    const int enabled = shapes_opt.get();
+    auto on = [&](int shape) { return shape >= 1 && shape <= 3 && ((enabled >> (shape - 1)) & 1) != 0; };
+    const int f_shape = shape_opt.get();
+    if (f_shape || !model_opt.get()) {
+        if (f_shape == 1 || (!f_shape && xl_tile_pays(p))) return on(1);
+        const long long wg_a = (((long long)p.height * p.width + 255) / 256) * (p.cout / 64);
+        return on((f_shape ? f_shape == 2 : wg_a >= 256) ? 2 : 3);
+    }
+    const PcChoice c = choose_pc_tile(p, pc_n_cu());
+    return on(c.shape) && (c.split_row == 0 || on(c.shape2));
 }
 
 constexpr double kPcExchangeUs = 25.0;
diff --git a/style-transfer-pytorch_amd/csrc/st_conv_split.hip b/style-transfer-pytorch_amd/csrc/st_conv_split.hip
--- a/style-transfer-pytorch_amd/csrc/st_conv_split.hip
+++ b/style-transfer-pytorch_amd/csrc/st_conv_split.hip
@@ -549,6 +549,8 @@
     ST_REQUIRE(p.cin % SK == 0 && p.cout % 64 == 0, "split conv: Cin %% 16 and Cout %% 64 required (got %d, %d)",
                p.cin, p.cout);
     ST_REQUIRE((long long)p.height * p.width * SK * 4 < (1ll << 30), "split conv: image too large");
+    ST_REQUIRE(!p.in_pool_code || conv_pooled_input_applies(p),
+               "split conv: no kernel with the pooled-input staging takes this problem (conv_pooled_input_applies)");
     const long long pixels = (long long)p.height * p.width;
     const int co_tiles = p.cout / 64;
     const long long wg_a = ((pixels + 255) / 256) * co_tiles, wg_b = ((pixels + 127) / 128) * co_tiles;
@@ -562,7 +564,7 @@
             ksplit *= 2;
     }
     if (p.elem == 1) {
-        if (p.amax_measure && launch_amax(p.in, (long long)p.cin * pixels, p.amax_word, 0, stream)) return 1;
+        if (p.amax_measure && launch_amax(p.in, (long long)p.cin * (p.in_pool_code ? pixels / 4 : pixels), p.amax_word, 0, stream)) return 1;
         if (!p.halo_amax_folded && fold_halo_amax(p, stream)) return 1;
         if (p.wgt_wino && p.wino && (p.wino > 1 ? conv_wino_applies(p) : conv_wino_preferred(p))) return launch_conv_wino(p, stream);
         if (conv_fat_preferred(p)) return launch_conv_fat(p, stream);
diff --git a/style-transfer-pytorch_amd/csrc/st_conv_wino.hip b/style-transfer-pytorch_amd/csrc/st_conv_wino.hip
--- a/style-transfer-pytorch_amd/csrc/st_conv_wino.hip
+++ b/style-transfer-pytorch_amd/csrc/st_conv_wino.hip
@@ -396,7 +396,9 @@
                 if (y1v[1] > m) { m = y1v[1]; at = 3; }
                 const int po = in1 ? poff0 + rr * (PH * PW * 4) : kOOR;
                 __builtin_amdgcn_raw_buffer_store_b32(__builtin_bit_cast(unsigned int, m), ps, po, 0, 0);
-                __builtin_amdgcn_raw_buffer_store_b8((unsigned char)(at | (m > 0.f ? 4 : 0)), cs, in1 ? (po >> 2) : kOOR, 0, 0);
+                const int cwin = ((oy >> 1) * PW + (ox >> 1)) * 8 + row0;
+                __builtin_amdgcn_raw_buffer_store_b8((unsigned char)(at | (m > 0.f ? 4 : 0)), cs,
+                                                     in1 ? cwin + (r >> 2) * (PH * PW * 8) + (r & 3) : kOOR, 0, 0);
             }
         }
     });
diff --git a/style-transfer-pytorch_amd/csrc/st_ops.hip b/style-transfer-pytorch_amd/csrc/st_ops.hip
--- a/style-transfer-pytorch_amd/csrc/st_ops.hip
+++ b/style-transfer-pytorch_amd/csrc/st_ops.hip
@@ -144,7 +144,7 @@
 static int conv_op(const float* in, const float* mask, const float* weight, const float* bias, float* out,
                    int cin, int cout, int height, int width, int relu, int dgrad, int precision, hipStream_t s,
                    const float* halo = nullptr, int has_up = 0, int has_down = 0, int accumulate = 0,
-                   const float* out_mask = nullptr, int overlap = 0) {
+                   const float* out_mask = nullptr, int overlap = 0, const unsigned char* in_codes = nullptr) {
     if (reject_winograd(precision)) return 1;
     const bool wino5 = precision == 5;
     if (wino5) precision = 4;
@@ -187,6 +187,11 @@
     c.in = in; c.mask = mask; c.wgt = wl; c.bias = bias; c.out = out; c.height = height; c.width = width;
     c.taps = 9; c.relu = relu; c.accumulate = accumulate; c.out_mask = out_mask;
     c.in_halo = halo; c.has_up = halo ? has_up : 0; c.has_down = halo ? has_down : 0;
+    if (in_codes) {
+        c.in_pool_code = in_codes;
+        ST_REQUIRE(conv_pooled_input_applies(c),
+                   "st_op_conv3x3_dgrad_pooled: no kernel with the pooled-input staging takes this problem (shape, precision or switches)");
+    }
     if (overlap) {
         PcOverlap o{};
         ST_REQUIRE(conv_pc_overlap_choice(c, &o), "st_op_conv3x3_strip_ex: this problem cannot be cut into interior + boundary launches");
@@ -348,6 +353,21 @@
                    static_cast<hipStream_t>(stream));
 }
 
+int st_op_conv3x3_dgrad_pooled(const float* grad_pooled, const unsigned char* codes, const float* weight, float* grad_in,
+                               const float* out_mask, int cin, int cout, int height, int width, int accumulate, void* stream) {
+    ST_REQUIRE(grad_pooled && codes && weight && grad_in, "st_op_conv3x3_dgrad_pooled: null argument");
+    ST_REQUIRE(height % 2 == 0 && width % 4 == 0 && cout % 16 == 0, "st_op_conv3x3_dgrad_pooled: even H, W %% 4 == 0, Cout %% 16 == 0 required");
+    return conv_op(grad_pooled, nullptr, weight, nullptr, grad_in, cin, cout, height, width, 0, 1, 4, static_cast<hipStream_t>(stream),
+                   nullptr, 0, 0, accumulate != 0, out_mask, 0, codes);
+}
+
+int st_op_pool2x2_backward_codes(const unsigned char* codes, const float* grad_out, float* grad_in, int channels, int height,
+                                 int width, void* stream) {
+    ST_REQUIRE(codes && grad_out && grad_in, "st_op_pool2x2_backward_codes: null argument");
+    ST_REQUIRE(channels > 0 && height >= 2 && width >= 4, "st_op_pool2x2_backward_codes: C >= 1, H >= 2, W >= 4 required");
+    return launch_pool_bwd_codes(codes, grad_out, grad_in, channels, height, width, static_cast<hipStream_t>(stream));
+}
+
 int st_op_conv3x3_strip(const float* in, const float* halo, int has_up, int has_down, const float* weight,
                         const float* bias, float* out, int cin, int cout, int height, int width, int relu, int dgrad,
                         int precision, void* stream) {
diff --git a/style-transfer-pytorch_amd/csrc/st_plan.h b/style-transfer-pytorch_amd/csrc/st_plan.h
--- a/style-transfer-pytorch_amd/csrc/st_plan.h
+++ b/style-transfer-pytorch_amd/csrc/st_plan.h
@@ -36,6 +36,7 @@
     bool pooled_by_conv = false;
     unsigned char* pool_code = nullptr;
     bool coded = false;
+    bool g_folded = false;
     unsigned int* y_amax = nullptr;
     unsigned int* g_amax = nullptr;
     size_t count() const { return (size_t)c * h * w; }
@@ -200,6 +201,7 @@
     hipEvent_t tl_h3[4] = {};
     int tl_count = 0;
     bool profiling = false;
+    long long pool_bwd_launched = 0, pool_bwd_folded = 0;
     std::vector<st::ProfileEvent> events;
     size_t events_used = 0;
     std::vector<st::HbmEvent> hbm_events;
diff --git a/style-transfer-pytorch_amd/csrc/st_pool.hip b/style-transfer-pytorch_amd/csrc/st_pool.hip
--- a/style-transfer-pytorch_amd/csrc/st_pool.hip
+++ b/style-transfer-pytorch_amd/csrc/st_pool.hip
@@ -150,30 +150,34 @@
 __global__ __launch_bounds__(256) void pool_bwd_codes_kernel(const unsigned char* __restrict__ code,
                                                              const float* __restrict__ gout, float* __restrict__ gin,
                                                              int C, int H, int W) {
-    const int Ho = H / 2, W4 = W / 4;
-    const long long total = (long long)C * Ho * W4;
+    typedef unsigned int u32x4 __attribute__((ext_vector_type(4)));
+    const int Ho = H / 2, Wo = W / 2, W4 = W / 4;
+    const long long total = (long long)(C / 8) * Ho * W4;
     for (long long i = blockIdx.x * 256ll + threadIdx.x; i < total; i += (long long)gridDim.x * 256) {
         const int x4 = (int)(i % W4);
         const long long row = i / W4;
         const int yo = (int)(row % Ho);
-        const long long c = row / Ho;
-        const size_t base = ((size_t)c * H + 2 * yo) * W + 4 * x4;
-        const size_t pooled = (size_t)row * (W / 2) + 2 * x4;
-        const unsigned short two = *reinterpret_cast<const unsigned short*>(code + pooled);
-        const f32x2 go = *reinterpret_cast<const f32x2*>(gout + pooled);
-        f32x4 g0 = {0.f, 0.f, 0.f, 0.f}, g1 = {0.f, 0.f, 0.f, 0.f};
+        const long long grp = row / Ho;
+        const u32x4 cds = *reinterpret_cast<const u32x4*>(code + ((size_t)row * Wo + 2 * x4) * 8);
 #pragma unroll
-        for (int w = 0; w < 2; ++w) {
-            const int cd = (two >> (8 * w)) & 0xff;
-            const float g = (cd & 4) ? go[w] : 0.f;
-            const int at = cd & 3;
-            g0[2 * w] = at == 0 ? g : 0.f;
-            g0[2 * w + 1] = at == 1 ? g : 0.f;
-            g1[2 * w] = at == 2 ? g : 0.f;
-            g1[2 * w + 1] = at == 3 ? g : 0.f;
+        for (int k = 0; k < 8; ++k) {
+            const size_t c = (size_t)grp * 8 + k;
+            const size_t base = (c * H + 2 * yo) * W + 4 * x4;
+            const f32x2 go = *reinterpret_cast<const f32x2*>(gout + (c * Ho + yo) * Wo + 2 * x4);
+            f32x4 g0 = {0.f, 0.f, 0.f, 0.f}, g1 = {0.f, 0.f, 0.f, 0.f};
+#pragma unroll
+            for (int w = 0; w < 2; ++w) {
+                const int cd = (cds[2 * w + (k >> 2)] >> (8 * (k & 3))) & 0xff;
+                const float g = (cd & 4) ? go[w] : 0.f;
+                const int at = cd & 3;
+                g0[2 * w] = at == 0 ? g : 0.f;
+                g0[2 * w + 1] = at == 1 ? g : 0.f;
+                g1[2 * w] = at == 2 ? g : 0.f;
+                g1[2 * w + 1] = at == 3 ? g : 0.f;
+            }
+            *reinterpret_cast<f32x4*>(gin + base) = g0;
+            *reinterpret_cast<f32x4*>(gin + base + W) = g1;
         }
-        *reinterpret_cast<f32x4*>(gin + base) = g0;
-        *reinterpret_cast<f32x4*>(gin + base + W) = g1;
     }
 }
 
@@ -181,8 +185,12 @@
 
 int launch_pool_bwd_codes(const unsigned char* code, const float* grad_out, float* grad_in, int channels, int height,
                           int width, hipStream_t s) {
-    ST_REQUIRE(width % 4 == 0 && height % 2 == 0, "pool backward from codes: W %% 4 == 0 and even H required");
-    const long long total4 = (long long)channels * (height / 2) * (width / 4);
+    ST_REQUIRE(width % 4 == 0 && height % 2 == 0 && channels % 8 == 0,
+               "pool backward from codes: W %% 4 == 0, even H and C %% 8 == 0 required");
+    ST_REQUIRE(((reinterpret_cast<uintptr_t>(code) | reinterpret_cast<uintptr_t>(grad_in)) & 15) == 0 &&
+                   (reinterpret_cast<uintptr_t>(grad_out) & 7) == 0,
+               "pool backward from codes: unaligned buffers");
+    const long long total4 = (long long)(channels / 8) * (height / 2) * (width / 4);
     const int blocks4 = (int)std::min<long long>((total4 + 255) / 256, 16384);
     hipLaunchKernelGGL(pool_bwd_codes_kernel, dim3(blocks4), dim3(256), 0, s, code, grad_out, grad_in, channels, height, width);
     ST_LAUNCH_CHECK();
diff --git a/style-transfer-pytorch_amd/style_transfer/_hip.py b/style-transfer-pytorch_amd/style_transfer/_hip.py
--- a/style-transfer-pytorch_amd/style_transfer/_hip.py
+++ b/style-transfer-pytorch_amd/style_transfer/_hip.py
@@ -103,6 +103,7 @@
         'st_plan_moment_sums': (i32, [vp, i32, vp, vp]),
         'st_plan_set_graph': (i32, [vp, i32]),
         'st_plan_profile_enable': (i32, [vp, i32]),
+        'st_plan_pool_backward_counts': (i32, [vp, ctypes.POINTER(i64), ctypes.POINTER(i64)]),
         'st_plan_profile_read': (i32, [vp, ctypes.POINTER(i64), ctypes.POINTER(f64), ctypes.POINTER(f64)]),
         'st_plan_profile_read_hbm': (i32, [vp, i32, ctypes.POINTER(i64), ctypes.POINTER(f64), ctypes.POINTER(f64)]),
         'st_op_sqrtm_ns': (i32, [vp, vp, i32, vp]),
@@ -118,6 +119,8 @@
         'st_op_conv3x3_time': (i32, [i32, i32, i32, i32, i32, i32, i32, ctypes.POINTER(f64), vp]),
         'st_op_conv3x3': (i32, [vp, vp, vp, vp, i32, i32, i32, i32, i32, i32, vp]),
         'st_op_conv3x3_dgrad': (i32, [vp, vp, vp, vp, i32, i32, i32, i32, i32, vp]),
+        'st_op_conv3x3_dgrad_pooled': (i32, [vp, vp, vp, vp, vp, i32, i32, i32, i32, i32, vp]),
+        'st_op_pool2x2_backward_codes': (i32, [vp, vp, vp, i32, i32, i32, vp]),
         'st_op_conv3x3_strip': (i32, [vp, vp, i32, i32, vp, vp, vp, i32, i32, i32, i32, i32, i32, i32, vp]),
         'st_op_conv3x3_strip_ex': (i32, [vp, vp, i32, i32, vp, vp, vp, vp, i32, i32, i32, i32, i32, i32, i32, i32, i32, vp]),
         'st_op_conv1x1': (i32, [vp, vp, vp, vp, i32, i32, i64, i32, vp]),
@@ -596,6 +599,11 @@
     def set_graph(self, on=True):
         _check(self.lib.st_plan_set_graph(self.handle, 1 if on else 0))
 
+    def pool_backward_counts(self):
+        a, b = ctypes.c_longlong(), ctypes.c_longlong()
+        _check(self.lib.st_plan_pool_backward_counts(self.handle, ctypes.byref(a), ctypes.byref(b)))
+        return a.value, b.value
+
     def profile_enable(self, on=True):
         _check(self.lib.st_plan_profile_enable(self.handle, 1 if on else 0))
 
@@ -959,6 +967,36 @@
     return gin
 
 
+def _code_ptr(codes):
+    assert codes.is_cuda and codes.dtype == torch.uint8 and codes.is_contiguous(), 'expected a contiguous uint8 HIP tensor'
+    return ctypes.c_void_p(codes.data_ptr())
+
+
+def op_pool2x2_backward_codes(codes, grad_out, height, width):
+    lib = load_library()
+    c = grad_out.shape[-3]
+    assert codes.numel() == c * (height // 2) * (width // 2) and grad_out.numel() == codes.numel()
+    grad_in = torch.empty((c, height, width), device=grad_out.device, dtype=torch.float32)
+    with torch.cuda.device(grad_out.device):
+        _check(lib.st_op_pool2x2_backward_codes(_code_ptr(codes), _ptr(grad_out.contiguous()), _ptr(grad_in), c, height, width,
+                                                _stream()))
+    return grad_in
+
+
+def op_conv3x3_dgrad_pooled(grad_pooled, codes, weight, height, width, out=None, out_mask=None):
+    lib = load_library()
+    cout, cin = weight.shape[:2]
+    assert grad_pooled.numel() == cout * (height // 2) * (width // 2) == codes.numel()
+    acc = out is not None
+    if out is None:
+        out = torch.empty((1, cin, height, width), device=grad_pooled.device, dtype=torch.float32)
+    with torch.cuda.device(grad_pooled.device):
+        _check(lib.st_op_conv3x3_dgrad_pooled(_ptr(grad_pooled.contiguous()), _code_ptr(codes), _ptr(weight.contiguous()), _ptr(out),
+                                              _ptr(out_mask.contiguous()) if out_mask is not None else None, cin, cout, height,
+                                              width, 1 if acc else 0, _stream()))
+    return out
+
+
 def _reduce_scratch(device):
     return torch.empty(int(load_library().st_op_reduce_scratch_floats()), device=device, dtype=torch.float32)
 
```

Result: no change. 437.3 it/s, median of 2 (+0.5%).
